# zhihu/ZhiLight

Measured on AMD Instinct MI355X. Metric: decode tokens/s (Llama-3-8B GPTQ-Int4, TP=1 per GPU, batch 1, seq 1024), higher is better.
Workload: dtype f16; 1 GPU; Llama-3-8B GPTQ-Int4 g128 TP=1 batch=1 decode seq=1024 (BASELINE configs[1]); layers=32, parallelism=dp1 (independent TP=1 replicas), global_batch=1, seq_len=1024, valid=True, kv_cache_dtype=fp16, w4_algo=mfma

## Files before the change

### zhilight_amd/build.py

```python
import os
import subprocess
import sys
from concurrent.futures import ThreadPoolExecutor

HERE = os.path.dirname(os.path.abspath(__file__))
CSRC = os.path.join(HERE, "csrc")
OUT = os.path.join(HERE, "libzhilight_amd.so")
HIPCC = os.environ.get("HIPCC", "/opt/rocm/bin/hipcc")
FLAGS = ["--offload-arch=gfx950", "-O3", "-std=c++17", "-fPIC", "-Wall", "-Wno-unused-function",
         "-fno-fast-math", "-ffp-contract=off"]
EXTRA_FLAGS = {"w4_slab.hip": ["-mllvm", "-pragma-unroll-threshold=200000"]}


EXPERIMENTAL = os.environ.get("ZL_BUILD_EXPERIMENTAL", "0") == "1"
EXPERIMENTAL_DIR = os.path.join(HERE, "..", "tools", "experimental")


def sources():
    srcs = sorted(os.path.join(CSRC, f) for f in os.listdir(CSRC) if f.endswith(".hip"))
    if EXPERIMENTAL:
        srcs.append(os.path.join(EXPERIMENTAL_DIR, "w4_engine.hip"))
    return srcs


def _stale(target, deps):
    if not os.path.exists(target):
        return True
    t = os.path.getmtime(target)
    return any(os.path.getmtime(d) > t for d in deps)


def build(force=False, verbose=False):
    srcs = sources()
    hdrs = [os.path.join(CSRC, f) for f in os.listdir(CSRC) if f.endswith(".h")]
    hdrs.append(os.path.join(HERE, "..", "include", "zhilight_amd.h"))
    objdir = os.path.join(HERE, "build")
    os.makedirs(objdir, exist_ok=True)
    flags = FLAGS + (["-DZL_EXPERIMENTAL", "-I" + CSRC] if EXPERIMENTAL else [])
    stamp = os.path.join(objdir, ".flags")
    if not os.path.exists(stamp) or open(stamp).read() != " ".join(flags):
        force = True
    objs = []
    jobs = []
    for s in srcs:
        o = os.path.join(objdir, os.path.basename(s)[:-4] + ".o")
        objs.append(o)
        if force or _stale(o, [s] + hdrs):
            jobs.append([HIPCC] + flags + EXTRA_FLAGS.get(os.path.basename(s), []) + ["-c", s, "-o", o])

    def run(cmd):
        if verbose:
            print(" ".join(cmd), flush=True)
        subprocess.check_call(cmd)

    with ThreadPoolExecutor(max_workers=min(8, max(1, len(jobs)))) as ex:
        list(ex.map(run, jobs))
    if jobs or force or _stale(OUT, objs):
        run([HIPCC, "--offload-arch=gfx950", "-shared", "-fPIC", "-o", OUT] + objs)
    with open(stamp, "w") as fh:
        fh.write(" ".join(flags))
    build_hostcpp(force, verbose)
    build_comm(force, verbose)
    _ref().build(force, verbose)
    return OUT


COMM_OUT = os.path.join(HERE, "libzhilight_amd_comm.so")


def build_comm(force=False, verbose=False):
    src = os.path.join(HERE, "csrc_comm", "comm.hip")
    deps = [src, os.path.join(HERE, "..", "include", "zhilight_amd_comm.h"), os.path.join(HERE, "..", "include", "zhilight_amd.h")]
    if not (force or _stale(COMM_OUT, deps)):
        return COMM_OUT
    rocm = os.environ.get("ROCM_PATH", "/opt/rocm")
    cmd = [HIPCC, "--offload-arch=gfx950", "-O3", "-std=c++17", "-fPIC", "-Wall", "-shared", "-o", COMM_OUT, src,
           "-L" + os.path.join(rocm, "lib"), "-lrccl"]
    if verbose:
        print(" ".join(cmd), flush=True)
    subprocess.check_call(cmd)
    return COMM_OUT


HOSTCPP = os.path.join(HERE, "hostcpp")


HOSTCPP_SOURCES = ("bm_hip.cpp", "bm_layer.cpp", "bm_functions.cpp", "bm_c10d.cpp", "nn_amd.cpp")
HOSTCPP_HEADERS = ("bm_hip.h", "bm_layer.h", "bm_functions.h", "bm_c10d.h", "nn_amd.h")


def hostcpp_target():
    import sysconfig
    return os.path.join(HERE, "zl_internals" + sysconfig.get_config_var("EXT_SUFFIX"))


def build_hostcpp(force=False, verbose=False):
    import pybind11
    import sysconfig
    srcs = [os.path.join(HOSTCPP, f) for f in HOSTCPP_SOURCES + ("py_internals.cpp",)]
    deps = srcs + [os.path.join(HOSTCPP, f) for f in HOSTCPP_HEADERS] + [os.path.join(HERE, "..", "include", "zhilight_amd.h")]
    target = hostcpp_target()
    if not (force or _stale(target, deps)):
        return target
    rocm = os.environ.get("ROCM_PATH", "/opt/rocm")
    cmd = [os.environ.get("CXX", "g++"), "-O2", "-std=c++17", "-fPIC", "-shared", "-D__HIP_PLATFORM_AMD__", "-I" + os.path.join(rocm, "include"),
           "-I" + os.path.join(HERE, "..", "include"), "-I" + pybind11.get_include(), "-I" + sysconfig.get_paths()["include"]] + srcs + [
           "-o", target, "-L" + HERE, "-lzhilight_amd", "-L" + os.path.join(rocm, "lib"), "-lamdhip64",
           "-Wl,-rpath,$ORIGIN", "-Wl,-rpath," + os.path.join(rocm, "lib")]
    if verbose:
        print(" ".join(cmd), flush=True)
    subprocess.check_call(cmd)
    return target


REFERENCE = os.environ.get("ZL_REFERENCE_ROOT", "/root/reference")
ORACLE = os.path.join(os.path.dirname(HERE), "oracle")
_REF_NAMES = ("REFDIR", "REF_TUS", "REF_CHECK_TUS", "REF_CHECK_NAMESPACES", "REF_REPORT_TUS", "REF_CHECK_PENDING",
              "REF_BINDING_TUS", "HOST_SOURCES", "HOST_HEADERS", "HARNESS_SOURCES", "host_target", "refcompile_target",
              "binding_target", "refcheck_report", "build_host", "build_refcompile", "build_binding", "build_refcheck")


def _ref():
    if ORACLE not in sys.path:
        sys.path.insert(0, ORACLE)
    import ref_build
    return ref_build


def __getattr__(name):
    if name in _REF_NAMES:
        return getattr(_ref(), name)
    raise AttributeError("module %r has no attribute %r" % (__name__, name))


if __name__ == "__main__":
    print(build(force="--force" in sys.argv, verbose=True))
```

### zhilight_amd/csrc/attention.hip

```cpp
#include <algorithm>
#include <type_traits>
#include "zl_common.h"

namespace {

constexpr int kSteps = 8;
constexpr int kMaxSplits = 512;

struct AttnParams {
    const uint16_t* q = nullptr;
    const int32_t* buf_lens = nullptr;
    const uint16_t* const* k_bufs = nullptr;
    const uint16_t* const* v_bufs = nullptr;
    const int8_t* mask = nullptr;
    const int32_t* valid_lens = nullptr;
    uint16_t* out = nullptr;
    float* ws = nullptr;
    int b = 0, len_q = 0, h = 0, hkv = 0, n_rep = 0, rows = 0;
    int passes = 0, split_len = 0, max_splits = 0;
    float scale = 0.f;
    int bshd = 0;
    const uint16_t* qkv = nullptr;
    const float* cosv = nullptr;
    const float* sinv = nullptr;
    const int32_t* placement = nullptr;
    uint16_t* const* k_bufs_w = nullptr;
    uint16_t* const* v_bufs_w = nullptr;
    int neox = 1;
    const float* const* k_scales = nullptr;
    const float* const* v_scales = nullptr;
    int half_partials = 0;
    int la = 0;
    int* la_cnt = nullptr;
    int causal = 0;
};

typedef _Float16 hv2 __attribute__((ext_vector_type(2)));

static inline int attn_split_len(int64_t b, int64_t hkv, int64_t max_len) {
    int64_t want = (max_len * b * hkv) / 1024;
    int64_t ls = (want / 128) * 128;
    if (ls < 128) ls = 128;
    if (ls <= 256 && ((max_len + ls - 1) / ls) * b * hkv > 1024) ls += 128;
    if (ls > 2048) ls = 2048;
    while ((max_len + ls - 1) / ls > kMaxSplits && ls < (int64_t)1 << 30) ls += 128;
    return (int)ls;
}

template <int DT>
__device__ __forceinline__ float dot8(const uint4& a, const uint4& b) {
    const uint32_t au[4] = {a.x, a.y, a.z, a.w}, bu[4] = {b.x, b.y, b.z, b.w};
    float acc = 0.f;
#pragma unroll
    for (int e = 0; e < 4; ++e) {
        if constexpr (DT == ZL_F16) {
            acc = __builtin_amdgcn_fdot2(__builtin_bit_cast(hv2, au[e]), __builtin_bit_cast(hv2, bu[e]), acc, false);
        } else {
            acc = __builtin_fmaf(__builtin_bit_cast(float, au[e] << 16), __builtin_bit_cast(float, bu[e] << 16), acc);
            acc = __builtin_fmaf(__builtin_bit_cast(float, au[e] & 0xffff0000u),
                                 __builtin_bit_cast(float, bu[e] & 0xffff0000u), acc);
        }
    }
    return acc;
}

template <int DT>
__device__ __forceinline__ void unpack8(const uint4& v, float (&f)[8]) {
    const uint32_t u[4] = {v.x, v.y, v.z, v.w};
#pragma unroll
    for (int e = 0; e < 4; ++e) {
        f[2 * e] = ZT<DT>::to_f32((uint16_t)(u[e] & 0xffff));
        f[2 * e + 1] = ZT<DT>::to_f32((uint16_t)(u[e] >> 16));
    }
}

template <int DT>
__device__ __forceinline__ uint4 rope8(const uint4& a, const uint4& b, const float* c, const float* s, int d0, int half,
                                       int neox) {
    float af[8], bf[8];
    unpack8<DT>(a, af);
    unpack8<DT>(b, bf);
    uint32_t o[4];
#pragma unroll
    for (int e = 0; e < 8; e += 2) {
        float r[2];
#pragma unroll
        for (int t = 0; t < 2; ++t) {
            const int i = e + t;
            bool minus;
            float partner;
            if (neox) {
                minus = (d0 + i) < half;
                partner = bf[i];
            } else {
                minus = (i & 1) == 0;
                partner = af[i ^ 1];
            }
            r[t] = minus ? __builtin_fmaf(-partner, s[i], af[i] * c[i]) : __builtin_fmaf(partner, s[i], af[i] * c[i]);
        }
        o[e / 2] = (uint32_t)ZT<DT>::from_f32(r[0]) | ((uint32_t)ZT<DT>::from_f32(r[1]) << 16);
    }
    return make_uint4(o[0], o[1], o[2], o[3]);
}

template <int LPK>
__device__ __forceinline__ float key_row_sum(float v) {
#ifdef ZL_ATTN_NO_DPP
#pragma unroll
    for (int off = LPK / 2; off > 0; off >>= 1) v += __shfl_xor(v, off, 64);
    return v;
#endif
    v += __builtin_bit_cast(float, __builtin_amdgcn_update_dpp(0, __builtin_bit_cast(int, v), 0xB1, 0xF, 0xF, false));
    v += __builtin_bit_cast(float, __builtin_amdgcn_update_dpp(0, __builtin_bit_cast(int, v), 0x4E, 0xF, 0xF, false));
    if (LPK >= 8)
        v += __builtin_bit_cast(float, __builtin_amdgcn_update_dpp(0, __builtin_bit_cast(int, v), 0x141, 0xF, 0xF, false));
    if (LPK >= 16)
        v += __builtin_bit_cast(float, __builtin_amdgcn_update_dpp(0, __builtin_bit_cast(int, v), 0x140, 0xF, 0xF, false));
    if (LPK >= 32) v += __shfl_xor(v, 16, 64);
    return v;
}

template <int DT, int D, int RT, bool FUSE, bool MASKED>
__global__ __launch_bounds__(256) void k_decode_attn_partial(const AttnParams p) {
    constexpr int LPK = D / 8;
    constexpr int KPS = 64 / LPK;
    constexpr int CHUNK = KPS * kSteps;
    __shared__ float xw[4][RT][D + 2];

    const int b = blockIdx.z / p.passes, pass = blockIdx.z % p.passes;
    const int hk = blockIdx.y, split = blockIdx.x;
    const int len = p.buf_lens[b];
    const int vlen_in = MASKED ? 0x7fffffff : p.valid_lens[b];
    const uint16_t* kbase = p.k_bufs[b];
    const uint16_t* vbase = p.v_bufs[b];
    const int place = FUSE ? p.placement[b] : -1;
    const int elen = MASKED ? len : min(len, vlen_in);
    const int t0 = split * p.split_len;
    const bool owns_new = FUSE && place >= t0 && place < t0 + p.split_len && place < len;
    if (t0 >= elen && !owns_new) return;
    const int t1 = min(elen, t0 + p.split_len);

    const int lane = threadIdx.x & 63, wave = threadIdx.x >> 6;
    const int grp = lane / LPK, dp = lane % LPK;
    const size_t kv_stride = p.bshd ? (size_t)p.hkv * D : (size_t)D;
    const size_t kv_off = (p.bshd ? (size_t)hk * D : (size_t)hk * len * D) + dp * 8;

    uint4 kk[kSteps], vv[kSteps];
    int c0 = t0 + wave * CHUNK;
    const int last_key = t1 > 0 ? t1 - 1 : 0;
#define ZL_LOAD_CHUNK(base)                                                                      \
    _Pragma("unroll") for (int st = 0; st < kSteps; ++st) {                                      \
        const int key_ = (base) + st * KPS + grp;                                                \
        const int kc_ = key_ < last_key ? key_ : last_key;                                       \
        kk[st] = *reinterpret_cast<const uint4*>(kbase + kv_off + (size_t)kc_ * kv_stride);     \
        vv[st] = *reinterpret_cast<const uint4*>(vbase + kv_off + (size_t)kc_ * kv_stride);     \
    }
    if (len <= 0) return;
    ZL_LOAD_CHUNK(c0)

    size_t mask_off = 0;
    if (MASKED) {
        for (int i = 0; i < b; ++i) mask_off += (size_t)p.buf_lens[i];
        mask_off *= p.len_q;
    }

    uint4 qv[RT];
    int q_of_row[RT];
    uint4 k_new = make_uint4(0, 0, 0, 0), v_new = make_uint4(0, 0, 0, 0);
    if constexpr (FUSE) {
        constexpr int half = D / 2;
        const int d0 = dp * 8;
        const int pd0 = p.neox ? (d0 < half ? d0 + half : d0 - half) : d0;
        float c[8], sn[8];
        const float4* cp = reinterpret_cast<const float4*>(p.cosv + (size_t)b * D + d0);
        const float4* sp = reinterpret_cast<const float4*>(p.sinv + (size_t)b * D + d0);
        const float4 c0v = cp[0], c1v = cp[1], s0v = sp[0], s1v = sp[1];
        c[0] = c0v.x; c[1] = c0v.y; c[2] = c0v.z; c[3] = c0v.w; c[4] = c1v.x; c[5] = c1v.y; c[6] = c1v.z; c[7] = c1v.w;
        sn[0] = s0v.x; sn[1] = s0v.y; sn[2] = s0v.z; sn[3] = s0v.w; sn[4] = s1v.x; sn[5] = s1v.y; sn[6] = s1v.z; sn[7] = s1v.w;
        const uint16_t* row = p.qkv + (size_t)b * (p.h + 2 * p.hkv) * D;
#pragma unroll
        for (int i = 0; i < RT; ++i) {
            qv[i] = make_uint4(0, 0, 0, 0);
            q_of_row[i] = 0;
            const int rr = pass * RT + i;
            if (rr < p.rows) {
                const uint16_t* src = row + (size_t)(hk * p.n_rep + rr) * D;
                qv[i] = rope8<DT>(*reinterpret_cast<const uint4*>(src + d0), *reinterpret_cast<const uint4*>(src + pd0), c, sn,
                                  d0, half, p.neox);
            }
        }
        const uint16_t* ksrc = row + (size_t)(p.h + hk) * D;
        k_new = rope8<DT>(*reinterpret_cast<const uint4*>(ksrc + d0), *reinterpret_cast<const uint4*>(ksrc + pd0), c, sn, d0,
                          half, p.neox);
        v_new = *reinterpret_cast<const uint4*>(row + (size_t)(p.h + p.hkv + hk) * D + d0);
        if (owns_new && pass == 0 && wave == 0 && grp == 0) {
            *reinterpret_cast<uint4*>(p.k_bufs_w[b] + kv_off + (size_t)place * kv_stride) = k_new;
            *reinterpret_cast<uint4*>(p.v_bufs_w[b] + kv_off + (size_t)place * kv_stride) = v_new;
        }
        if (t0 >= elen) return;
    } else {
#pragma unroll
        for (int i = 0; i < RT; ++i) {
            const int rr = pass * RT + i;
            qv[i] = make_uint4(0, 0, 0, 0);
            q_of_row[i] = 0;
            if (rr < p.rows) {
                const int qi = rr / p.n_rep, head = hk * p.n_rep + rr % p.n_rep;
                q_of_row[i] = qi;
                qv[i] = *reinterpret_cast<const uint4*>(p.q + (((size_t)b * p.len_q + qi) * p.h + head) * D + dp * 8);
            }
        }
    }

    float m[RT], l[RT], acc[RT][8];
#pragma unroll
    for (int i = 0; i < RT; ++i) {
        m[i] = -1e20f;
        l[i] = 0.f;
#pragma unroll
        for (int e = 0; e < 8; ++e) acc[i][e] = 0.f;
    }

    while (c0 < t1) {
        float sc[RT][kSteps];
#pragma unroll
        for (int st = 0; st < kSteps; ++st) {
            const int key = c0 + st * KPS + grp;
            if (FUSE && key == place) {
                kk[st] = k_new;
                vv[st] = v_new;
            }
            const bool inb = key < t1;
#pragma unroll
            for (int i = 0; i < RT; ++i) {
                const float d = key_row_sum<LPK>(dot8<DT>(qv[i], kk[st]));
                bool vis = inb;
                if (MASKED) {
                    if (vis) vis = p.mask[mask_off + (size_t)q_of_row[i] * len + key] != 0;
                }
                sc[i][st] = vis ? d * p.scale : -INFINITY;
            }
            if (!inb) vv[st] = make_uint4(0, 0, 0, 0);
        }
#pragma unroll
        for (int i = 0; i < RT; ++i) {
            float mc = sc[i][0];
#pragma unroll
            for (int st = 1; st < kSteps; ++st) mc = fmaxf(mc, sc[i][st]);
            const float mn = fmaxf(m[i], mc);
            const float alpha = __expf(m[i] - mn);
            m[i] = mn;
            l[i] *= alpha;
#pragma unroll
            for (int e = 0; e < 8; ++e) acc[i][e] *= alpha;
        }
#pragma unroll
        for (int st = 0; st < kSteps; ++st) {
            float vf[8];
            unpack8<DT>(vv[st], vf);
            if (MASKED) {
                bool any = false;
#pragma unroll
                for (int i = 0; i < RT; ++i) any = any || (sc[i][st] != -INFINITY);
                if (!any) {
#pragma unroll
                    for (int e = 0; e < 8; ++e) vf[e] = 0.f;
                }
            }
#pragma unroll
            for (int i = 0; i < RT; ++i) {
                const float pr = __expf(sc[i][st] - m[i]);
                l[i] += pr;
#pragma unroll
                for (int e = 0; e < 8; ++e) acc[i][e] = __builtin_fmaf(pr, vf[e], acc[i][e]);
            }
        }
        c0 += 4 * CHUNK;
        if (c0 >= t1) break;
        ZL_LOAD_CHUNK(c0)
    }
#undef ZL_LOAD_CHUNK

#pragma unroll
    for (int off = LPK; off < 64; off <<= 1) {
#pragma unroll
        for (int i = 0; i < RT; ++i) {
            const float m2 = __shfl_xor(m[i], off, 64), l2 = __shfl_xor(l[i], off, 64);
            const float mn = fmaxf(m[i], m2);
            const float f1 = __expf(m[i] - mn), f2 = __expf(m2 - mn);
            l[i] = l[i] * f1 + l2 * f2;
#pragma unroll
            for (int e = 0; e < 8; ++e) {
                const float a2 = __shfl_xor(acc[i][e], off, 64);
                acc[i][e] = acc[i][e] * f1 + a2 * f2;
            }
            m[i] = mn;
        }
    }
    if (grp == 0) {
#pragma unroll
        for (int i = 0; i < RT; ++i) {
#pragma unroll
            for (int e = 0; e < 8; ++e) xw[wave][i][dp * 8 + e] = acc[i][e];
            if (dp == 0) {
                xw[wave][i][D] = m[i];
                xw[wave][i][D + 1] = l[i];
            }
        }
    }
    __syncthreads();
    for (int idx = threadIdx.x; idx < RT * D; idx += 256) {
        const int i = idx / D, d = idx % D;
        const int rr = pass * RT + i;
        if (rr >= p.rows) continue;
        float mn = xw[0][i][D];
#pragma unroll
        for (int w = 1; w < 4; ++w) mn = fmaxf(mn, xw[w][i][D]);
        float a = 0.f, lt = 0.f;
#pragma unroll
        for (int w = 0; w < 4; ++w) {
            const float f = __expf(xw[w][i][D] - mn);
            a = __builtin_fmaf(xw[w][i][d], f, a);
            lt = __builtin_fmaf(xw[w][i][D + 1], f, lt);
        }
        const int qi = rr / p.n_rep, head = hk * p.n_rep + rr % p.n_rep;
        float* dst = p.ws + ((((size_t)b * p.len_q + qi) * p.h + head) * p.max_splits + split) * (D + 2);
        dst[d] = a;
        if (d == 0) {
            dst[D] = mn;
            dst[D + 1] = lt;
        }
    }
}

__device__ __forceinline__ void codes_to_h2(const uint4& w, hv2 (&h)[8]) {
    const uint32_t u[4] = {w.x, w.y, w.z, w.w};
    const hv2 bias = {(_Float16)1152.f, (_Float16)1152.f};
#pragma unroll
    for (int e = 0; e < 4; ++e) {
        h[2 * e] = __builtin_bit_cast(hv2, __builtin_amdgcn_perm(0x64646464u, u[e], 0x04010400u)) - bias;
        h[2 * e + 1] = __builtin_bit_cast(hv2, __builtin_amdgcn_perm(0x64646464u, u[e], 0x04030402u)) - bias;
    }
}
__device__ __forceinline__ void codes_to_f32(const uint4& w, float (&f)[16]) {
    const uint32_t u[4] = {w.x, w.y, w.z, w.w};
#pragma unroll
    for (int e = 0; e < 4; ++e) {
#pragma unroll
        for (int j = 0; j < 4; ++j) f[4 * e + j] = (float)((u[e] >> (8 * j)) & 0xffu) - 128.f;
    }
}

template <int DT, int D, int RT, bool MASKED>
__global__ __launch_bounds__(256) void k_decode_attn_partial_q8(const AttnParams p) {
    constexpr int LPK = D / 16;
    constexpr int KPS = 64 / LPK;
    constexpr int CHUNK = KPS * kSteps;
    constexpr int QW = DT == ZL_F16 ? 8 : 16;
    __shared__ float xw[4][RT][D + 2];

    const int b = blockIdx.z / p.passes, pass = blockIdx.z % p.passes;
    const int hk = blockIdx.y, split = blockIdx.x;
    const int len = p.buf_lens[b];
    const int vlen_in = MASKED ? 0x7fffffff : p.valid_lens[b];
    const uint8_t* kbase = reinterpret_cast<const uint8_t*>(p.k_bufs[b]);
    const uint8_t* vbase = reinterpret_cast<const uint8_t*>(p.v_bufs[b]);
    const float* ksc = p.k_scales[b];
    const float* vsc = p.v_scales[b];
    const int elen = MASKED ? len : min(len, vlen_in);
    const int t0 = split * p.split_len;
    if (t0 >= elen || len <= 0) return;
    const int t1 = min(elen, t0 + p.split_len);

    const int lane = threadIdx.x & 63, wave = threadIdx.x >> 6;
    const int grp = lane / LPK, dp = lane % LPK;
    const size_t kv_stride = p.bshd ? (size_t)p.hkv * D : (size_t)D;
    const size_t kv_off = (p.bshd ? (size_t)hk * D : (size_t)hk * len * D) + dp * 16;
    const size_t sc_stride = p.bshd ? (size_t)p.hkv : 1;
    const size_t sc_off = p.bshd ? (size_t)hk : (size_t)hk * len;

    uint4 kk[kSteps], vv[kSteps];
    float ks[kSteps], vs[kSteps];
    int c0 = t0 + wave * CHUNK;
    const int last_key = t1 - 1;
#define ZL_LOAD_CHUNK_Q8(base)                                                                   \
    _Pragma("unroll") for (int st = 0; st < kSteps; ++st) {                                      \
        const int key_ = (base) + st * KPS + grp;                                                \
        const int kc_ = key_ < last_key ? key_ : last_key;                                       \
        kk[st] = *reinterpret_cast<const uint4*>(kbase + kv_off + (size_t)kc_ * kv_stride);     \
        vv[st] = *reinterpret_cast<const uint4*>(vbase + kv_off + (size_t)kc_ * kv_stride);     \
        ks[st] = ksc[sc_off + (size_t)kc_ * sc_stride];                                          \
        vs[st] = vsc[sc_off + (size_t)kc_ * sc_stride];                                          \
    }
    ZL_LOAD_CHUNK_Q8(c0)

    size_t mask_off = 0;
    if (MASKED) {
        for (int i = 0; i < b; ++i) mask_off += (size_t)p.buf_lens[i];
        mask_off *= p.len_q;
    }

    hv2 qh[RT][8];
    float qf[RT][QW];
    int q_of_row[RT];
#pragma unroll
    for (int i = 0; i < RT; ++i) {
        const int rr = pass * RT + i;
        uint4 lo = make_uint4(0, 0, 0, 0), hi = lo;
        q_of_row[i] = 0;
        if (rr < p.rows) {
            const int qi = rr / p.n_rep, head = hk * p.n_rep + rr % p.n_rep;
            q_of_row[i] = qi;
            const uint16_t* qp = p.q + (((size_t)b * p.len_q + qi) * p.h + head) * D + dp * 16;
            lo = *reinterpret_cast<const uint4*>(qp);
            hi = *reinterpret_cast<const uint4*>(qp + 8);
        }
        if constexpr (DT == ZL_F16) {
            const uint32_t u[8] = {lo.x, lo.y, lo.z, lo.w, hi.x, hi.y, hi.z, hi.w};
#pragma unroll
            for (int e = 0; e < 8; ++e) qh[i][e] = __builtin_bit_cast(hv2, u[e]);
        } else {
            float a[8], c[8];
            unpack8<DT>(lo, a);
            unpack8<DT>(hi, c);
#pragma unroll
            for (int e = 0; e < 8; ++e) {
                qf[i][e] = a[e];
                qf[i][8 + e] = c[e];
            }
        }
    }

    float m[RT], l[RT], acc[RT][16];
#pragma unroll
    for (int i = 0; i < RT; ++i) {
        m[i] = -1e20f;
        l[i] = 0.f;
#pragma unroll
        for (int e = 0; e < 16; ++e) acc[i][e] = 0.f;
    }

    while (c0 < t1) {
        float sc[RT][kSteps];
#pragma unroll
        for (int st = 0; st < kSteps; ++st) {
            const int key = c0 + st * KPS + grp;
            const bool inb = key < t1;
            const float lscale = ks[st] * p.scale;
            hv2 kh[8];
            float kf[16];
            if constexpr (DT == ZL_F16) codes_to_h2(kk[st], kh);
            else codes_to_f32(kk[st], kf);
#pragma unroll
            for (int i = 0; i < RT; ++i) {
                float d = 0.f;
                if constexpr (DT == ZL_F16) {
#pragma unroll
                    for (int e = 0; e < 8; ++e) d = __builtin_amdgcn_fdot2(qh[i][e], kh[e], d, false);
                } else {
#pragma unroll
                    for (int e = 0; e < 16; ++e) d = __builtin_fmaf(qf[i][e], kf[e], d);
                }
                d = key_row_sum<LPK>(d);
                bool vis = inb;
                if (MASKED) {
                    if (vis) vis = p.mask[mask_off + (size_t)q_of_row[i] * len + key] != 0;
                }
                sc[i][st] = vis ? d * lscale : -INFINITY;
            }
            if (!inb) vs[st] = 0.f;
        }
#pragma unroll
        for (int i = 0; i < RT; ++i) {
            float mc = sc[i][0];
#pragma unroll
            for (int st = 1; st < kSteps; ++st) mc = fmaxf(mc, sc[i][st]);
            const float mn = fmaxf(m[i], mc);
            const float alpha = __expf(m[i] - mn);
            m[i] = mn;
            l[i] *= alpha;
#pragma unroll
            for (int e = 0; e < 16; ++e) acc[i][e] *= alpha;
        }
#pragma unroll
        for (int st = 0; st < kSteps; ++st) {
            float vf[16];
            codes_to_f32(vv[st], vf);
            float sv = vs[st];
            if (MASKED) {
                bool any = false;
#pragma unroll
                for (int i = 0; i < RT; ++i) any = any || (sc[i][st] != -INFINITY);
                if (!any) sv = 0.f;
            }
#pragma unroll
            for (int i = 0; i < RT; ++i) {
                const float pr = __expf(sc[i][st] - m[i]);
                l[i] += pr;
                const float w = pr * sv;
#pragma unroll
                for (int e = 0; e < 16; ++e) acc[i][e] = __builtin_fmaf(w, vf[e], acc[i][e]);
            }
        }
        c0 += 4 * CHUNK;
        if (c0 >= t1) break;
        ZL_LOAD_CHUNK_Q8(c0)
    }
#undef ZL_LOAD_CHUNK_Q8

#pragma unroll
    for (int off = LPK; off < 64; off <<= 1) {
#pragma unroll
        for (int i = 0; i < RT; ++i) {
            const float m2 = __shfl_xor(m[i], off, 64), l2 = __shfl_xor(l[i], off, 64);
            const float mn = fmaxf(m[i], m2);
            const float f1 = __expf(m[i] - mn), f2 = __expf(m2 - mn);
            l[i] = l[i] * f1 + l2 * f2;
#pragma unroll
            for (int e = 0; e < 16; ++e) {
                const float a2 = __shfl_xor(acc[i][e], off, 64);
                acc[i][e] = acc[i][e] * f1 + a2 * f2;
            }
            m[i] = mn;
        }
    }
    if (grp == 0) {
#pragma unroll
        for (int i = 0; i < RT; ++i) {
#pragma unroll
            for (int e = 0; e < 16; ++e) xw[wave][i][dp * 16 + e] = acc[i][e];
            if (dp == 0) {
                xw[wave][i][D] = m[i];
                xw[wave][i][D + 1] = l[i];
            }
        }
    }
    __syncthreads();
    for (int idx = threadIdx.x; idx < RT * D; idx += 256) {
        const int i = idx / D, d = idx % D;
        const int rr = pass * RT + i;
        if (rr >= p.rows) continue;
        float mn = xw[0][i][D];
#pragma unroll
        for (int w = 1; w < 4; ++w) mn = fmaxf(mn, xw[w][i][D]);
        float a = 0.f, lt = 0.f;
#pragma unroll
        for (int w = 0; w < 4; ++w) {
            const float f = __expf(xw[w][i][D] - mn);
            a = __builtin_fmaf(xw[w][i][d], f, a);
            lt = __builtin_fmaf(xw[w][i][D + 1], f, lt);
        }
        const int qi = rr / p.n_rep, head = hk * p.n_rep + rr % p.n_rep;
        float* dst = p.ws + ((((size_t)b * p.len_q + qi) * p.h + head) * p.max_splits + split) * (D + 2);
        dst[d] = a;
        if (d == 0) {
            dst[D] = mn;
            dst[D + 1] = lt;
        }
    }
}

typedef _Float16 h8v __attribute__((ext_vector_type(8)));
typedef float f4v __attribute__((ext_vector_type(4)));
typedef short s4v __attribute__((ext_vector_type(4)));
constexpr int kMD = 128;
constexpr int kMVS = kMD + 16;

template <int DT>
__device__ __forceinline__ f4v mfma_t(uint4 a, uint4 b, f4v c) {
    typedef __bf16 b8v __attribute__((ext_vector_type(8)));
    if constexpr (DT == ZL_F16)
        return __builtin_amdgcn_mfma_f32_16x16x32_f16(__builtin_bit_cast(h8v, a), __builtin_bit_cast(h8v, b), c, 0, 0, 0);
    else
        return __builtin_amdgcn_mfma_f32_16x16x32_bf16(__builtin_bit_cast(b8v, a), __builtin_bit_cast(b8v, b), c, 0, 0, 0);
}

#ifndef ZL_LA_BATCH
#define ZL_LA_BATCH 16
#endif
constexpr int kLaBatch = ZL_LA_BATCH;
#ifdef ZL_ATTN_PROBE
__device__ unsigned long long* zl_aprobe_p = nullptr;
#define ZL_APROBE_INIT()                                                                                           \
    unsigned long long* ap_ = nullptr;                                                                             \
    {                                                                                                              \
        const unsigned wg_ = (blockIdx.z * gridDim.y + blockIdx.y) * gridDim.x + blockIdx.x;                        \
        if (zl_aprobe_p && (threadIdx.x & 63) == 0 && wg_ < 8192) ap_ = zl_aprobe_p + ((size_t)wg_ * 8 + (threadIdx.x >> 6)) * 8; \
    }
#define ZL_APROBE(slot) do { if (ap_) ap_[slot] = wall_clock64(); } while (0)
#else
#define ZL_APROBE_INIT() do {} while (0)
#define ZL_APROBE(slot) do {} while (0)
#endif
constexpr int kLaMaxSplits = 64;

template <int DT>
__device__ __forceinline__ void attn_tail_la(const AttnParams& p, float* xw, int b, int hk, int split, int nw, int ns, unsigned long long* ap_) {
    (void)ap_;
    constexpr int WS = 16 * (kMD + 2);
    const int nthr = nw * 64;
    const bool direct = ns == 1;
    const size_t stat0 = (size_t)p.b * p.len_q * p.h * p.max_splits * (kMD / 2);
    for (int it = threadIdx.x; it < p.rows * (kMD / 4); it += nthr) {
        const int i = it / (kMD / 4), d0 = (it % (kMD / 4)) * 4;
        const float* src = xw + (size_t)i * (kMD + 2);
        float mn = src[kMD];
        for (int w = 1; w < nw; ++w) mn = fmaxf(mn, src[w * WS + kMD]);
        float a[4] = {0.f, 0.f, 0.f, 0.f}, lt = 0.f;
        for (int w = 0; w < nw; ++w) {
            const float f = __expf(src[w * WS + kMD] - mn);
            typedef float f2v __attribute__((ext_vector_type(2)));
            const f2v v01 = *reinterpret_cast<const f2v*>(src + w * WS + d0), v23 = *reinterpret_cast<const f2v*>(src + w * WS + d0 + 2);
            const f4v v = (f4v){v01[0], v01[1], v23[0], v23[1]};
#pragma unroll
            for (int e = 0; e < 4; ++e) a[e] = __builtin_fmaf(v[e], f, a[e]);
            lt = __builtin_fmaf(src[w * WS + kMD + 1], f, lt);
        }
        const int qi = i / p.n_rep, head = hk * p.n_rep + i % p.n_rep;
        const size_t vh = ((size_t)b * p.len_q + qi) * p.h + head;
        const size_t rec = vh * p.max_splits + split;
        if (direct) {
            uint16_t o4[4];
#pragma unroll
            for (int e = 0; e < 4; ++e) {
                float ov;
                if (p.half_partials) ov = ((float)(_Float16)(a[e] / lt) * lt) * (1.0f / (lt + 1e-20f));
                else ov = a[e] / (lt + 1e-20f);
                o4[e] = ZT<DT>::from_f32(ov);
            }
            *reinterpret_cast<uint2*>(p.out + vh * kMD + d0) = make_uint2((uint32_t)o4[0] | ((uint32_t)o4[1] << 16), (uint32_t)o4[2] | ((uint32_t)o4[3] << 16));
            continue;
        }
        auto st8 = [](void* dst, uint32_t lo, uint32_t hi) {
            __hip_atomic_store(reinterpret_cast<uint64_t*>(dst), (uint64_t)lo | ((uint64_t)hi << 32), __ATOMIC_RELAXED, __HIP_MEMORY_SCOPE_AGENT);
        };
        if (p.half_partials) {
            uint32_t w2[2];
#pragma unroll
            for (int e = 0; e < 2; ++e)
                w2[e] = (uint32_t)__builtin_bit_cast(uint16_t, (_Float16)(a[2 * e] / lt)) | ((uint32_t)__builtin_bit_cast(uint16_t, (_Float16)(a[2 * e + 1] / lt)) << 16);
            st8(reinterpret_cast<uint16_t*>(p.ws) + rec * kMD + d0, w2[0], w2[1]);
            if (d0 == 0) st8(p.ws + stat0 + rec * 2, __builtin_bit_cast(uint32_t, mn), __builtin_bit_cast(uint32_t, lt));
        } else {
            float* dst = p.ws + rec * (kMD + 2) + d0;
            st8(dst, __builtin_bit_cast(uint32_t, a[0]), __builtin_bit_cast(uint32_t, a[1]));
            st8(dst + 2, __builtin_bit_cast(uint32_t, a[2]), __builtin_bit_cast(uint32_t, a[3]));
            if (d0 == 0) st8(dst + kMD, __builtin_bit_cast(uint32_t, mn), __builtin_bit_cast(uint32_t, lt));
        }
    }
    if (direct) return;
#if defined(__HIP_DEVICE_COMPILE__) && !defined(__gfx950__)
#error "attn_tail_la's hand-off is written for gfx950 (vmcnt-tracked write-through stores); revisit it for any other target"
#endif
    asm volatile("s_waitcnt vmcnt(0)" ::: "memory");
    __syncthreads();
    ZL_APROBE(5);
    int* flag = reinterpret_cast<int*>(xw);
    if (threadIdx.x == 0) {
        int* cnt = p.la_cnt + (size_t)b * p.hkv + hk;
        const int old = __hip_atomic_fetch_add(cnt, 1, __ATOMIC_RELAXED, __HIP_MEMORY_SCOPE_AGENT);
        if (old == ns - 1) __hip_atomic_store(cnt, 0, __ATOMIC_RELAXED, __HIP_MEMORY_SCOPE_AGENT);
        *flag = old == ns - 1;
    }
    __syncthreads();
    ZL_APROBE(6);
    if (!*flag) return;
    for (int it = threadIdx.x; it < p.rows * (kMD / 4); it += nthr) {
        const int i = it / (kMD / 4), d0 = (it % (kMD / 4)) * 4;
        const int qi = i / p.n_rep, head = hk * p.n_rep + i % p.n_rep;
        const size_t vh = ((size_t)b * p.len_q + qi) * p.h + head;
        float mn = -1e20f, a[4] = {0.f, 0.f, 0.f, 0.f}, z = 0.f;
        for (int u0 = 0; u0 < ns; u0 += kLaBatch) {
            uint64_t lo[kLaBatch], hi[kLaBatch], ml[kLaBatch];
#pragma unroll
            for (int j = 0; j < kLaBatch; ++j) {
                const size_t rec = vh * p.max_splits + min(u0 + j, ns - 1);
                if (p.half_partials) {
                    lo[j] = __hip_atomic_load(reinterpret_cast<const uint64_t*>(reinterpret_cast<const uint16_t*>(p.ws) + (rec * kMD + d0)),
                                              __ATOMIC_RELAXED, __HIP_MEMORY_SCOPE_AGENT);
                    hi[j] = 0;
                    ml[j] = __hip_atomic_load(reinterpret_cast<const uint64_t*>(p.ws + stat0 + rec * 2), __ATOMIC_RELAXED, __HIP_MEMORY_SCOPE_AGENT);
                } else {
                    const uint64_t* src = reinterpret_cast<const uint64_t*>(p.ws + rec * (kMD + 2) + d0);
                    lo[j] = __hip_atomic_load(src, __ATOMIC_RELAXED, __HIP_MEMORY_SCOPE_AGENT);
                    hi[j] = __hip_atomic_load(src + 1, __ATOMIC_RELAXED, __HIP_MEMORY_SCOPE_AGENT);
                    ml[j] = __hip_atomic_load(reinterpret_cast<const uint64_t*>(p.ws + rec * (kMD + 2) + kMD), __ATOMIC_RELAXED, __HIP_MEMORY_SCOPE_AGENT);
                }
            }
            float mb = mn;
#pragma unroll
            for (int j = 0; j < kLaBatch; ++j)
                if (u0 + j < ns) mb = fmaxf(mb, __builtin_bit_cast(float, (uint32_t)ml[j]));
            if (u0 > 0) {
                const float r = __expf(mn - mb);
#pragma unroll
                for (int e = 0; e < 4; ++e) a[e] *= r;
                z *= r;
            }
            mn = mb;
#pragma unroll
            for (int j = 0; j < kLaBatch; ++j) {
                if (u0 + j < ns) {
                    const float ms = __builtin_bit_cast(float, (uint32_t)ml[j]), ls = __builtin_bit_cast(float, (uint32_t)(ml[j] >> 32));
                    if (p.half_partials) {
                        const float f = ls * __expf(ms - mn);
#pragma unroll
                        for (int e = 0; e < 4; ++e)
                            a[e] = __builtin_fmaf((float)__builtin_bit_cast(_Float16, (uint16_t)(lo[j] >> (16 * e))), f, a[e]);
                        z += f;
                    } else {
                        const float f = __expf(ms - mn);
                        a[0] = __builtin_fmaf(__builtin_bit_cast(float, (uint32_t)lo[j]), f, a[0]);
                        a[1] = __builtin_fmaf(__builtin_bit_cast(float, (uint32_t)(lo[j] >> 32)), f, a[1]);
                        a[2] = __builtin_fmaf(__builtin_bit_cast(float, (uint32_t)hi[j]), f, a[2]);
                        a[3] = __builtin_fmaf(__builtin_bit_cast(float, (uint32_t)(hi[j] >> 32)), f, a[3]);
                        z = __builtin_fmaf(ls, f, z);
                    }
                }
            }
        }
        uint16_t o4[4];
        const float zi = 1.0f / (z + 1e-20f);
#pragma unroll
        for (int e = 0; e < 4; ++e) o4[e] = ZT<DT>::from_f32(p.half_partials ? a[e] * zi : a[e] / (z + 1e-20f));
        *reinterpret_cast<uint2*>(p.out + vh * kMD + d0) = make_uint2((uint32_t)o4[0] | ((uint32_t)o4[1] << 16), (uint32_t)o4[2] | ((uint32_t)o4[3] << 16));
    }
    ZL_APROBE(7);
}

#ifndef ZL_ATTN8_WAVES_PER_SIMD
#define ZL_ATTN8_WAVES_PER_SIMD 2
#endif
#define ZL_ATTN8_OCC(NW_) ((NW_) == 4 ? 4 : ZL_ATTN8_WAVES_PER_SIMD)
template <int DT, int NW = 4, bool LA = false, int PF = 1, bool MASKED = false, bool CAUSAL = false>
__global__ __launch_bounds__(64 * NW, PF >= 3 ? 1 : (PF == 2 || MASKED) ? 2 : ZL_ATTN8_OCC(NW)) void k_decode_attn_mfma(const AttnParams p) {
    static_assert(!MASKED || (!LA && PF == 1), "the mask form exists for the two-launch route only");
    static_assert(!CAUSAL || (!LA && PF == 1 && !MASKED && NW == 4), "the causal form exists for the two-launch route only");
    __shared__ __attribute__((aligned(16))) uint16_t vs[NW][32 * kMVS];
    const int b = blockIdx.z, hk = CAUSAL ? (int)(blockIdx.y % (unsigned)p.hkv) : (int)blockIdx.y, split = blockIdx.x;
    const int row0 = CAUSAL ? 16 * (int)(blockIdx.y / (unsigned)p.hkv) : 0;
    const int nrows = CAUSAL ? min(16, p.rows - row0) : p.rows;
    const int len = p.buf_lens[b];
    const int vlen_in = MASKED ? 0x7fffffff : CAUSAL ? p.valid_lens[b] + (row0 + nrows - 1) / p.n_rep : p.valid_lens[b];
    const int8_t* mrow = nullptr;
    if constexpr (MASKED) {
        size_t mask_off = 0;
        for (int i = 0; i < b; ++i) mask_off += (size_t)p.buf_lens[i];
        mrow = p.mask + mask_off;
    }
    const uint16_t* kbase = p.k_bufs[b];
    const uint16_t* vbase = p.v_bufs[b];
    const int elen = min(len, vlen_in);
    const int t0 = split * p.split_len;
    const int nw = LA ? __builtin_amdgcn_readfirstlane((int)(blockDim.x >> 6)) : NW;
    ZL_APROBE_INIT();
    ZL_APROBE(0);
    if (t0 >= elen || len <= 0) {
        if constexpr (LA) {
            if (split == 0)
                for (int idx = threadIdx.x; idx < p.rows * kMD; idx += nw * 64) {
                    const int i = idx / kMD, qi = i / p.n_rep, head = hk * p.n_rep + i % p.n_rep;
                    p.out[(((size_t)b * p.len_q + qi) * p.h + head) * kMD + idx % kMD] = 0;
                }
        }
        return;
    }
    const int t1 = min(elen, t0 + p.split_len);
    const int last_key = t1 - 1;

    const int lane = threadIdx.x & 63, wave = threadIdx.x >> 6;
    const int r = lane & 15, kq = lane >> 4;
    const size_t kv_stride = p.bshd ? (size_t)p.hkv * kMD : (size_t)kMD;
    const size_t kv_off = p.bshd ? (size_t)hk * kMD : (size_t)hk * len * kMD;

    uint4 kkA[2][4], kkB[PF >= 2 ? 2 : 1][4], kkC[PF >= 3 ? 2 : 1][4];
    uint4 vA0, vA1, vA2, vA3, vA4, vA5, vA6, vA7, vB0, vB1, vB2, vB3, vB4, vB5, vB6, vB7, vC0, vC1, vC2, vC3, vC4, vC5, vC6, vC7;
    int c0 = t0 + wave * 32;
    const int cstep = nw * 32;
#define ZL_MFMA_LOAD_K(KK, base)                                                                                  \
    _Pragma("unroll") for (int blk_ = 0; blk_ < 2; ++blk_) {                                                   \
        const int key_ = (base) + 16 * blk_ + r;                                                               \
        const uint16_t* src_ = kbase + kv_off + (size_t)(key_ < last_key ? key_ : last_key) * kv_stride + 8 * kq; \
        _Pragma("unroll") for (int t_ = 0; t_ < 4; ++t_) KK[blk_][t_] = *reinterpret_cast<const uint4*>(src_ + 32 * t_); \
    }
#define ZL_MFMA_V1(VS, j_, base)                                                                                 \
    {                                                                                                          \
        const int key_ = (base) + 4 * j_ + (lane >> 4);                                                        \
        VS##j_ = *reinterpret_cast<const uint4*>(vbase + kv_off + (size_t)(key_ < last_key ? key_ : last_key) * kv_stride + (lane & 15) * 8); \
    }
#define ZL_MFMA_LOAD_V(VS, base)                                                                               \
    ZL_MFMA_V1(VS, 0, base) ZL_MFMA_V1(VS, 1, base) ZL_MFMA_V1(VS, 2, base) ZL_MFMA_V1(VS, 3, base) ZL_MFMA_V1(VS, 4, base) \
    ZL_MFMA_V1(VS, 5, base) ZL_MFMA_V1(VS, 6, base) ZL_MFMA_V1(VS, 7, base)
    int mbA = 1, mbX = 1;
#define ZL_MFMA_LOAD_M(MB, base)                                                                               \
    if constexpr (MASKED) {                                                                                    \
        const int key_ = (base) + (lane & 31);                                                                 \
        MB = mrow[key_ < last_key ? key_ : last_key];                                                          \
    }
    ZL_MFMA_LOAD_M(mbA, c0)
    ZL_MFMA_LOAD_K(kkA, c0)
    ZL_MFMA_LOAD_V(vA, c0)
    if constexpr (PF >= 2) {
        ZL_MFMA_LOAD_K(kkB, c0 + cstep)
        ZL_MFMA_LOAD_V(vB, c0 + cstep)
    }
    if constexpr (PF >= 3) {
        ZL_MFMA_LOAD_K(kkC, c0 + 2 * cstep)
        ZL_MFMA_LOAD_V(vC, c0 + 2 * cstep)
    }
    ZL_APROBE(1);

    uint4 qf[4];
    int rlim = t1;
    {
        uint4 z = make_uint4(0, 0, 0, 0);
        const bool live = r < nrows;
        const int rr = row0 + (live ? r : 0);
        const int qi = rr / p.n_rep, head = hk * p.n_rep + rr % p.n_rep;
        if constexpr (CAUSAL) rlim = min(t1, p.valid_lens[b] + qi);
        const uint16_t* qp = p.q + (((size_t)b * p.len_q + qi) * p.h + head) * kMD + 8 * kq;
#pragma unroll
        for (int t = 0; t < 4; ++t) {
            uint4 v = *reinterpret_cast<const uint4*>(qp + 32 * t);
            qf[t] = live ? v : z;
        }
    }

    f4v o[8];
#pragma unroll
    for (int db = 0; db < 8; ++db) o[db] = (f4v){0.f, 0.f, 0.f, 0.f};
    float m_run = -1e20f, l_run = 0.f;
    uint16_t* vsw = vs[wave];
    const uint16_t* vtr = vsw + (4 * kq + (r >> 2)) * kMVS + 4 * (r & 3);

    if (c0 >= t1) c0 = -1;
    auto chunk = [&](uint4 (&KK)[2][4], uint4& v0, uint4& v1, uint4& v2, uint4& v3, uint4& v4, uint4& v5, uint4& v6, uint4& v7,
                     int& MB, const int cur) __attribute__((always_inline)) {
        uint32_t vbits = 0xffffffffu;
        if constexpr (MASKED) {
            vbits = (uint32_t)__ballot(lane < 32 && MB != 0 && cur + lane < t1);
            const int vsh = lane >> 4;
#define ZL_MFMA_VZ(j_) if (!((vbits >> (4 * j_ + vsh)) & 1u)) v##j_ = make_uint4(0, 0, 0, 0);
            ZL_MFMA_VZ(0) ZL_MFMA_VZ(1) ZL_MFMA_VZ(2) ZL_MFMA_VZ(3) ZL_MFMA_VZ(4) ZL_MFMA_VZ(5) ZL_MFMA_VZ(6) ZL_MFMA_VZ(7)
#undef ZL_MFMA_VZ
        }
        f4v st[2];
#pragma unroll
        for (int blk = 0; blk < 2; ++blk) {
            st[blk] = (f4v){0.f, 0.f, 0.f, 0.f};
#pragma unroll
            for (int t = 0; t < 4; ++t)
                st[blk] = mfma_t<DT>(KK[blk][t], qf[t], st[blk]);
        }
        {
            uint16_t* vdst = vsw + (lane >> 4) * kMVS + (lane & 15) * 8;
#define ZL_MFMA_VST(j_) *reinterpret_cast<uint4*>(vdst + 4 * j_ * kMVS) = v##j_;
            ZL_MFMA_VST(0) ZL_MFMA_VST(1) ZL_MFMA_VST(2) ZL_MFMA_VST(3) ZL_MFMA_VST(4) ZL_MFMA_VST(5) ZL_MFMA_VST(6) ZL_MFMA_VST(7)
#undef ZL_MFMA_VST
        }
        ZL_MFMA_LOAD_M(MB, cur + PF * cstep)
        ZL_MFMA_LOAD_K(KK, cur + PF * cstep)
        ZL_MFMA_LOAD_V(v, cur + PF * cstep)
        float sv[2][4];
        float mloc = -INFINITY;
#pragma unroll
        for (int blk = 0; blk < 2; ++blk) {
#pragma unroll
            for (int i = 0; i < 4; ++i) {
                const int key = cur + 16 * blk + 4 * kq + i;
                bool vis = key < (CAUSAL ? rlim : t1);
                if constexpr (MASKED) vis = (vbits >> (16 * blk + 4 * kq + i)) & 1u;
                sv[blk][i] = vis ? st[blk][i] * p.scale : -INFINITY;
                mloc = fmaxf(mloc, sv[blk][i]);
            }
        }
        mloc = fmaxf(mloc, __shfl_xor(mloc, 16, 64));
        mloc = fmaxf(mloc, __shfl_xor(mloc, 32, 64));
        const float m_new = fmaxf(m_run, mloc);
        const float alpha = __expf(m_run - m_new);
#ifdef ZL_ATTN_PROBE
        if (m_run == -1e20f && m_new > -1e19f) ZL_APROBE(2);
#endif
        m_run = m_new;
        float pr[2][4];
        float lsum = 0.f;
#pragma unroll
        for (int blk = 0; blk < 2; ++blk) {
#pragma unroll
            for (int i = 0; i < 4; ++i) {
                pr[blk][i] = __expf(sv[blk][i] - m_new);
                lsum += pr[blk][i];
            }
        }
        auto cvt = [](float x) -> uint16_t {
            if constexpr (DT == ZL_F16) return __builtin_bit_cast(uint16_t, (_Float16)x);
            else {
                uint32_t u = __builtin_bit_cast(uint32_t, x);
                return (uint16_t)((u + 0x7fffu + ((u >> 16) & 1u)) >> 16);
            }
        };
        auto hi_lo = [&](float a, float b2, uint32_t& hw, uint32_t& lw) {
            const uint16_t ah = cvt(a), bh = cvt(b2);
            hw = (uint32_t)ah | ((uint32_t)bh << 16);
            lw = (uint32_t)cvt(a - ZT<DT>::to_f32(ah)) | ((uint32_t)cvt(b2 - ZT<DT>::to_f32(bh)) << 16);
        };
        uint4 pf, pl;
        hi_lo(pr[0][0], pr[0][1], pf.x, pl.x);
        hi_lo(pr[0][2], pr[0][3], pf.y, pl.y);
        hi_lo(pr[1][0], pr[1][1], pf.z, pl.z);
        hi_lo(pr[1][2], pr[1][3], pf.w, pl.w);
        l_run = l_run * alpha + lsum;
#pragma unroll
        for (int db = 0; db < 8; ++db) {
            o[db][0] *= alpha; o[db][1] *= alpha; o[db][2] *= alpha; o[db][3] *= alpha;
        }
#pragma unroll
        for (int db = 0; db < 8; ++db) {
            const s4v lo = __builtin_amdgcn_ds_read_tr16_b64_v4i16((__attribute__((address_space(3))) s4v*)(vtr + 16 * db));
            const s4v hi = __builtin_amdgcn_ds_read_tr16_b64_v4i16((__attribute__((address_space(3))) s4v*)(vtr + 16 * kMVS + 16 * db));
            typedef short s8v __attribute__((ext_vector_type(8)));
            const s8v a = __builtin_shufflevector(lo, hi, 0, 1, 2, 3, 4, 5, 6, 7);
            o[db] = mfma_t<DT>(__builtin_bit_cast(uint4, a), pf, o[db]);
            o[db] = mfma_t<DT>(__builtin_bit_cast(uint4, a), pl, o[db]);
        }
    };
    while (c0 >= 0) {
        chunk(kkA, vA0, vA1, vA2, vA3, vA4, vA5, vA6, vA7, mbA, c0);
        c0 += cstep;
        if (c0 >= t1) break;
        if constexpr (PF >= 2) {
            chunk(kkB, vB0, vB1, vB2, vB3, vB4, vB5, vB6, vB7, mbX, c0);
            c0 += cstep;
            if (c0 >= t1) break;
        }
        if constexpr (PF >= 3) {
            chunk(kkC, vC0, vC1, vC2, vC3, vC4, vC5, vC6, vC7, mbX, c0);
            c0 += cstep;
            if (c0 >= t1) break;
        }
    }
#undef ZL_MFMA_LOAD_K
#undef ZL_MFMA_LOAD_V
#undef ZL_MFMA_LOAD_M
#undef ZL_MFMA_V1

    ZL_APROBE(3);
    l_run += __shfl_xor(l_run, 16, 64);
    l_run += __shfl_xor(l_run, 32, 64);
    __syncthreads();
    float* xw = reinterpret_cast<float*>(&vs[0][0]);
    if (r < nrows) {
        float* dst = xw + ((size_t)wave * 16 + r) * (kMD + 2);
#pragma unroll
        for (int db = 0; db < 8; ++db) *reinterpret_cast<f4v*>(dst + 16 * db + 4 * kq) = o[db];
        if (kq == 0) {
            dst[kMD] = m_run;
            dst[kMD + 1] = l_run;
        }
    }
    __syncthreads();
    if constexpr (LA) {
        ZL_APROBE(4);
#ifdef ZL_ATTN_PROBE
        attn_tail_la<DT>(p, xw, b, hk, split, nw, (elen + p.split_len - 1) / p.split_len, ap_);
#else
        attn_tail_la<DT>(p, xw, b, hk, split, nw, (elen + p.split_len - 1) / p.split_len, nullptr);
#endif
        return;
    }
    for (int idx = threadIdx.x; idx < nrows * kMD; idx += NW * 64) {
        const int i = idx / kMD, d = idx % kMD;
        const float* src = xw + (size_t)i * (kMD + 2);
        constexpr int WS = 16 * (kMD + 2);
        float mn = src[kMD];
#pragma unroll
        for (int w = 1; w < NW; ++w) mn = fmaxf(mn, src[w * WS + kMD]);
        float a = 0.f, lt = 0.f;
#pragma unroll
        for (int w = 0; w < NW; ++w) {
            const float f = __expf(src[w * WS + kMD] - mn);
            a = __builtin_fmaf(src[w * WS + d], f, a);
            lt = __builtin_fmaf(src[w * WS + kMD + 1], f, lt);
        }
        const int qi = (row0 + i) / p.n_rep, head = hk * p.n_rep + (row0 + i) % p.n_rep;
        const size_t rec = (((size_t)b * p.len_q + qi) * p.h + head) * p.max_splits + split;
        if (p.half_partials) {
            uint16_t* hp = reinterpret_cast<uint16_t*>(p.ws);
            hp[rec * kMD + d] = __builtin_bit_cast(uint16_t, (_Float16)((MASKED && lt == 0.f) ? 0.f : a / lt));
            if (d == 0) {
                float* st = p.ws + (size_t)p.b * p.len_q * p.h * p.max_splits * (kMD / 2) + rec * 2;
                st[0] = mn;
                st[1] = lt;
            }
            continue;
        }
        float* dst = p.ws + rec * (kMD + 2);
        dst[d] = a;
        if (d == 0) {
            dst[kMD] = mn;
            dst[kMD + 1] = lt;
        }
    }
}

__global__ __launch_bounds__(256, 3) void k_decode_attn_mfma_q8(const AttnParams p) {
    __shared__ __attribute__((aligned(16))) uint16_t vs[4][32 * kMVS];
    const int b = blockIdx.z, hk = blockIdx.y, split = blockIdx.x;
    const int len = p.buf_lens[b];
    const int vlen_in = p.valid_lens[b];
    const uint8_t* kbase = reinterpret_cast<const uint8_t*>(p.k_bufs[b]);
    const uint8_t* vbase = reinterpret_cast<const uint8_t*>(p.v_bufs[b]);
    const float* ksc = p.k_scales[b];
    const float* vsc = p.v_scales[b];
    const int elen = min(len, vlen_in);
    const int t0 = split * p.split_len;
    if (t0 >= elen || len <= 0) return;
    const int t1 = min(elen, t0 + p.split_len);
    const int last_key = t1 - 1;

    const int lane = threadIdx.x & 63, wave = threadIdx.x >> 6;
    const int r = lane & 15, kq = lane >> 4;
    const size_t kv_stride = p.bshd ? (size_t)p.hkv * kMD : (size_t)kMD;
    const size_t kv_off = p.bshd ? (size_t)hk * kMD : (size_t)hk * len * kMD;
    const size_t sc_stride = p.bshd ? (size_t)p.hkv : 1;
    const size_t sc_off = p.bshd ? (size_t)hk : (size_t)hk * len;

    uint4 kk[2][2], vv0, vv1, vv2, vv3;
    float ksv[2][4], vsv[2][4];
    int c0 = t0 + wave * 32;
#define ZL_Q8_LOAD_K(base)                                                                                     \
    _Pragma("unroll") for (int blk_ = 0; blk_ < 2; ++blk_) {                                                   \
        const int key_ = (base) + 16 * blk_ + r;                                                               \
        const uint8_t* src_ = kbase + kv_off + (size_t)(key_ < last_key ? key_ : last_key) * kv_stride + 16 * kq; \
        kk[blk_][0] = *reinterpret_cast<const uint4*>(src_);                                                   \
        kk[blk_][1] = *reinterpret_cast<const uint4*>(src_ + 64);                                              \
        _Pragma("unroll") for (int i_ = 0; i_ < 4; ++i_) {                                                     \
            const int ks_ = (base) + 16 * blk_ + 4 * kq + i_;                                                  \
            const size_t so_ = sc_off + (size_t)(ks_ < last_key ? ks_ : last_key) * sc_stride;                 \
            ksv[blk_][i_] = ksc[so_];                                                                          \
            vsv[blk_][i_] = vsc[so_];                                                                          \
        }                                                                                                      \
    }
#define ZL_Q8_V1(j_, base)                                                                                     \
    {                                                                                                          \
        const int key_ = (base) + 8 * j_ + (lane >> 3);                                                        \
        vv##j_ = *reinterpret_cast<const uint4*>(vbase + kv_off + (size_t)(key_ < last_key ? key_ : last_key) * kv_stride + (lane & 7) * 16); \
    }
#define ZL_Q8_LOAD_V(base) ZL_Q8_V1(0, base) ZL_Q8_V1(1, base) ZL_Q8_V1(2, base) ZL_Q8_V1(3, base)
    ZL_Q8_LOAD_K(c0)
    ZL_Q8_LOAD_V(c0)

    h8v qf[4];
    {
        uint4 z = make_uint4(0, 0, 0, 0);
        const bool live = r < p.rows;
        const int rr = live ? r : 0;
        const int qi = rr / p.n_rep, head = hk * p.n_rep + rr % p.n_rep;
        const uint16_t* qp = p.q + (((size_t)b * p.len_q + qi) * p.h + head) * kMD + 16 * kq;
#pragma unroll
        for (int t = 0; t < 4; ++t) {
            uint4 v = *reinterpret_cast<const uint4*>(qp + 64 * (t >> 1) + 8 * (t & 1));
            qf[t] = __builtin_bit_cast(h8v, live ? v : z);
        }
    }

    f4v o[8];
#pragma unroll
    for (int db = 0; db < 8; ++db) o[db] = (f4v){0.f, 0.f, 0.f, 0.f};
    float m_run = -1e20f, l_run = 0.f;
    uint16_t* vsw = vs[wave];
    const uint16_t* vtr = vsw + (4 * kq + (r >> 2)) * kMVS + 4 * (r & 3);
    const hv2 bias = {(_Float16)1152.f, (_Float16)1152.f};
    auto cvt8 = [&](uint32_t w0, uint32_t w1) {
        uint4 o4;
        o4.x = __builtin_bit_cast(uint32_t, __builtin_bit_cast(hv2, __builtin_amdgcn_perm(0x64646464u, w0, 0x04010400u)) - bias);
        o4.y = __builtin_bit_cast(uint32_t, __builtin_bit_cast(hv2, __builtin_amdgcn_perm(0x64646464u, w0, 0x04030402u)) - bias);
        o4.z = __builtin_bit_cast(uint32_t, __builtin_bit_cast(hv2, __builtin_amdgcn_perm(0x64646464u, w1, 0x04010400u)) - bias);
        o4.w = __builtin_bit_cast(uint32_t, __builtin_bit_cast(hv2, __builtin_amdgcn_perm(0x64646464u, w1, 0x04030402u)) - bias);
        return o4;
    };

    if (c0 >= t1) c0 = -1;
    while (c0 >= 0) {
        f4v st[2];
        float ks_cur[2][4], vs_cur[2][4];
#pragma unroll
        for (int blk = 0; blk < 2; ++blk) {
            st[blk] = (f4v){0.f, 0.f, 0.f, 0.f};
#pragma unroll
            for (int u = 0; u < 2; ++u) {
                const uint4 c = kk[blk][u];
                st[blk] = __builtin_amdgcn_mfma_f32_16x16x32_f16(__builtin_bit_cast(h8v, cvt8(c.x, c.y)), qf[2 * u], st[blk], 0, 0, 0);
                st[blk] = __builtin_amdgcn_mfma_f32_16x16x32_f16(__builtin_bit_cast(h8v, cvt8(c.z, c.w)), qf[2 * u + 1], st[blk], 0, 0, 0);
            }
#pragma unroll
            for (int i = 0; i < 4; ++i) {
                ks_cur[blk][i] = ksv[blk][i];
                vs_cur[blk][i] = vsv[blk][i];
            }
        }
        {
            uint16_t* vdst = vsw + (lane >> 3) * kMVS + (lane & 7) * 16;
#define ZL_Q8_VST(j_)                                                                                          \
            *reinterpret_cast<uint4*>(vdst + 8 * j_ * kMVS) = cvt8(vv##j_.x, vv##j_.y);                        \
            *reinterpret_cast<uint4*>(vdst + 8 * j_ * kMVS + 8) = cvt8(vv##j_.z, vv##j_.w);
            ZL_Q8_VST(0) ZL_Q8_VST(1) ZL_Q8_VST(2) ZL_Q8_VST(3)
#undef ZL_Q8_VST
        }
        const int cur = c0;
        c0 += 4 * 32;
        ZL_Q8_LOAD_K(c0)
        ZL_Q8_LOAD_V(c0)
        float sv[2][4];
        float mloc = -INFINITY;
#pragma unroll
        for (int blk = 0; blk < 2; ++blk) {
#pragma unroll
            for (int i = 0; i < 4; ++i) {
                const int key = cur + 16 * blk + 4 * kq + i;
                sv[blk][i] = key < t1 ? st[blk][i] * (ks_cur[blk][i] * p.scale) : -INFINITY;
                mloc = fmaxf(mloc, sv[blk][i]);
            }
        }
        mloc = fmaxf(mloc, __shfl_xor(mloc, 16, 64));
        mloc = fmaxf(mloc, __shfl_xor(mloc, 32, 64));
        const float m_new = fmaxf(m_run, mloc);
        const float alpha = __expf(m_run - m_new);
        m_run = m_new;
        h8v pf, pl;
        float lsum = 0.f;
#pragma unroll
        for (int blk = 0; blk < 2; ++blk) {
#pragma unroll
            for (int i = 0; i < 4; ++i) {
                const int key = cur + 16 * blk + 4 * kq + i;
                const float pr = __expf(sv[blk][i] - m_new);
                lsum += pr;
                const float pw = key < t1 ? pr * vs_cur[blk][i] : 0.f;
                const _Float16 ph = (_Float16)pw;
                pf[blk * 4 + i] = ph;
                pl[blk * 4 + i] = (_Float16)(pw - (float)ph);
            }
        }
        l_run = l_run * alpha + lsum;
#pragma unroll
        for (int db = 0; db < 8; ++db) {
            o[db][0] *= alpha; o[db][1] *= alpha; o[db][2] *= alpha; o[db][3] *= alpha;
        }
#pragma unroll
        for (int db = 0; db < 8; ++db) {
            const s4v lo = __builtin_amdgcn_ds_read_tr16_b64_v4i16((__attribute__((address_space(3))) s4v*)(vtr + 16 * db));
            const s4v hi = __builtin_amdgcn_ds_read_tr16_b64_v4i16((__attribute__((address_space(3))) s4v*)(vtr + 16 * kMVS + 16 * db));
            typedef short s8v __attribute__((ext_vector_type(8)));
            const s8v a = __builtin_shufflevector(lo, hi, 0, 1, 2, 3, 4, 5, 6, 7);
            o[db] = __builtin_amdgcn_mfma_f32_16x16x32_f16(__builtin_bit_cast(h8v, a), pf, o[db], 0, 0, 0);
            o[db] = __builtin_amdgcn_mfma_f32_16x16x32_f16(__builtin_bit_cast(h8v, a), pl, o[db], 0, 0, 0);
        }
        if (c0 >= t1) break;
    }
#undef ZL_Q8_LOAD_K
#undef ZL_Q8_LOAD_V
#undef ZL_Q8_V1

    l_run += __shfl_xor(l_run, 16, 64);
    l_run += __shfl_xor(l_run, 32, 64);
    __syncthreads();
    float* xw = reinterpret_cast<float*>(&vs[0][0]);
    if (r < p.rows) {
        float* dst = xw + ((size_t)wave * 16 + r) * (kMD + 2);
#pragma unroll
        for (int db = 0; db < 8; ++db) *reinterpret_cast<f4v*>(dst + 16 * db + 4 * kq) = o[db];
        if (kq == 0) {
            dst[kMD] = m_run;
            dst[kMD + 1] = l_run;
        }
    }
    __syncthreads();
    for (int idx = threadIdx.x; idx < p.rows * kMD; idx += 256) {
        const int i = idx / kMD, d = idx % kMD;
        const float* src = xw + (size_t)i * (kMD + 2);
        constexpr int WS = 16 * (kMD + 2);
        float mn = src[kMD];
#pragma unroll
        for (int w = 1; w < 4; ++w) mn = fmaxf(mn, src[w * WS + kMD]);
        float a = 0.f, lt = 0.f;
#pragma unroll
        for (int w = 0; w < 4; ++w) {
            const float f = __expf(src[w * WS + kMD] - mn);
            a = __builtin_fmaf(src[w * WS + d], f, a);
            lt = __builtin_fmaf(src[w * WS + kMD + 1], f, lt);
        }
        const int qi = i / p.n_rep, head = hk * p.n_rep + i % p.n_rep;
        float* dst = p.ws + ((((size_t)b * p.len_q + qi) * p.h + head) * p.max_splits + split) * (kMD + 2);
        dst[d] = a;
        if (d == 0) {
            dst[kMD] = mn;
            dst[kMD + 1] = lt;
        }
    }
}

template <int DT, int D>
__global__ void k_decode_attn_combine(const AttnParams p) {
    constexpr int kMaxS = 512;
    __shared__ float sf[kMaxS];
    __shared__ float red[16];
    const int vh = blockIdx.x;
    const int b = vh / (p.len_q * p.h);
    const int len = p.buf_lens[b];
    const int vlen_in = p.valid_lens ? p.valid_lens[b] + (p.causal ? (vh / p.h) % p.len_q : 0) : 0x7fffffff;
    const int elen = p.mask ? len : min(len, vlen_in);
    const int ns = min((elen + p.split_len - 1) / p.split_len, kMaxS);
    const int d = threadIdx.x;
    const float* src = p.ws + (size_t)vh * p.max_splits * (D + 2);
    if (ns <= 16) {
        float v[16];
#pragma unroll
        for (int u = 0; u < 16; ++u) v[u] = src[(size_t)min(u, max(ns - 1, 0)) * (D + 2) + d];
        if (d < ns) {
            sf[d] = src[(size_t)d * (D + 2) + D];
            sf[64 + d] = src[(size_t)d * (D + 2) + D + 1];
        }
        __syncthreads();
        float mn = -1e20f;
        for (int s = 0; s < ns; ++s) mn = fmaxf(mn, sf[s]);
        float a = 0.f, z = 0.f;
#pragma unroll
        for (int u = 0; u < 16; ++u) {
            if (u < ns) {
                const float f = __expf(sf[u] - mn);
                a = __builtin_fmaf(v[u], f, a);
                z = __builtin_fmaf(sf[64 + u], f, z);
            }
        }
        p.out[(size_t)vh * D + d] = ZT<DT>::from_f32(a / (z + 1e-20f));
        return;
    }
    float mloc = -1e20f;
    for (int s = d; s < ns; s += D) {
        const float ms = src[(size_t)s * (D + 2) + D];
        sf[s] = ms;
        mloc = fmaxf(mloc, ms);
    }
    const float mn = zl_block_max(mloc, red);
    float zloc = 0.f;
    for (int s = d; s < ns; s += D) {
        const float f = __expf(sf[s] - mn);
        sf[s] = f;
        zloc = __builtin_fmaf(src[(size_t)s * (D + 2) + D + 1], f, zloc);
    }
    const float z = zl_block_sum(zloc, red);
    float a = 0.f;
    int s = 0;
    for (; s + 4 <= ns; s += 4) {
        const float v0 = src[(size_t)(s + 0) * (D + 2) + d], v1 = src[(size_t)(s + 1) * (D + 2) + d];
        const float v2 = src[(size_t)(s + 2) * (D + 2) + d], v3 = src[(size_t)(s + 3) * (D + 2) + d];
        a = __builtin_fmaf(v0, sf[s], a);
        a = __builtin_fmaf(v1, sf[s + 1], a);
        a = __builtin_fmaf(v2, sf[s + 2], a);
        a = __builtin_fmaf(v3, sf[s + 3], a);
    }
    for (; s < ns; ++s) a = __builtin_fmaf(src[(size_t)s * (D + 2) + d], sf[s], a);
    p.out[(size_t)vh * D + d] = ZT<DT>::from_f32(a / (z + 1e-20f));
}

__global__ __launch_bounds__(kMD) void k_decode_attn_combine_h(const AttnParams p) {
    const int vh = blockIdx.x, b = vh / p.h, d = threadIdx.x;
    const int len = p.buf_lens[b];
    const int elen = p.valid_lens ? min(len, p.valid_lens[b]) : len;
    const int ns = min((elen + p.split_len - 1) / p.split_len, p.max_splits);
    const uint16_t* part = reinterpret_cast<const uint16_t*>(p.ws) + (size_t)vh * p.max_splits * kMD;
    const float2* stat = reinterpret_cast<const float2*>(p.ws + (size_t)p.b * p.h * p.max_splits * (kMD / 2)) + (size_t)vh * p.max_splits;
    float mn = -1e20f;
    for (int u = 0; u < ns; ++u) mn = fmaxf(mn, stat[u].x);
    float a = 0.f, z = 0.f;
    for (int u = 0; u < ns; ++u) {
        const float2 st = stat[u];
        const float f = st.y * __expf(st.x - mn);
        a = __builtin_fmaf((float)__builtin_bit_cast(_Float16, part[(size_t)u * kMD + d]), f, a);
        z += f;
    }
    const float zi = 1.0f / (z + 1e-20f);
    p.out[(size_t)vh * kMD + d] = __builtin_bit_cast(uint16_t, zl_f32_to_f16(a * zi));
}

#define ZL_ATTN_TRY(...)                 \
    do {                                \
        const int e_ = (__VA_ARGS__);   \
        if (e_) return e_;              \
    } while (0)

template <class F>
static inline int by_dtype(int dtype, F&& f) {
    return dtype == ZL_F16 ? f(std::integral_constant<int, ZL_F16>{}) : f(std::integral_constant<int, ZL_BF16>{});
}

static inline int attn_check_args(bool pointers, int64_t b, int64_t len_q, int64_t h, int64_t hkv, int64_t d, int64_t max_len_buf) {
    ZL_CHECK_ARG(pointers, ZL_EINVAL);
    ZL_CHECK_ARG(b > 0 && len_q > 0 && h > 0 && hkv > 0 && d > 0 && max_len_buf > 0, ZL_EINVAL);
    ZL_CHECK_ARG(h % hkv == 0, ZL_ESHAPE);
    return ZL_OK;
}

static inline bool attn_dtype_ok(int dtype) { return dtype == ZL_F16 || dtype == ZL_BF16; }

static inline bool attn_mfma_shape_ok(int64_t b, int64_t h, int64_t hkv, int64_t d) {
    return d == kMD && h / hkv <= 16 && b <= 65535 && hkv <= 65535;
}

static int attn_geometry(AttnParams& p, int64_t b, int64_t len_q, int64_t h, int64_t hkv, int64_t max_len_buf,
                         int cap = kMaxSplits, int split_len = 0) {
    p.b = (int)b; p.len_q = (int)len_q; p.h = (int)h; p.hkv = (int)hkv; p.n_rep = (int)(h / hkv);
    p.rows = p.len_q * p.n_rep;
    p.split_len = split_len ? split_len : attn_split_len(b, hkv, max_len_buf);
    p.max_splits = (int)((max_len_buf + p.split_len - 1) / p.split_len);
    return p.max_splits <= cap ? ZL_OK : ZL_ELIMIT;
}

static int attn_set_passes(AttnParams& p, int rt) {
    p.passes = (p.rows + rt - 1) / rt;
    return (int64_t)p.b * p.passes <= 65535 && p.hkv <= 65535 ? ZL_OK : ZL_ELIMIT;
}

template <int NW = 4, bool LA = false, int PF = 1, bool MASKED = false, bool CAUSAL = false>
int launch_mfma(const AttnParams& p, int dtype, hipStream_t st, int waves = NW) {
    const int tiles = CAUSAL ? (p.rows + 15) / 16 : 1;
    const dim3 grid((unsigned)p.max_splits, (unsigned)(p.hkv * tiles), (unsigned)p.b);
    return by_dtype(dtype, [&](auto dt) {
        hipLaunchKernelGGL((k_decode_attn_mfma<decltype(dt)::value, NW, LA, PF, MASKED, CAUSAL>), grid, dim3(64 * waves), 0, st, p);
        return zl_launch_status();
    });
}

template <int D>
int launch_combine(const AttnParams& p, int dtype, hipStream_t st) {
    return by_dtype(dtype, [&](auto dt) {
        hipLaunchKernelGGL((k_decode_attn_combine<decltype(dt)::value, D>), dim3((unsigned)((int64_t)p.b * p.len_q * p.h)), dim3(D), 0, st, p);
        return zl_launch_status();
    });
}

static inline int valu_rt(int rows) { return rows >= 8 ? 8 : (rows >= 4 ? 4 : (rows >= 2 ? 2 : 1)); }
static inline int q8_rt(int rows) { return rows >= 4 ? 4 : (rows >= 2 ? 2 : 1); }

template <int DT, int D, bool FUSE>
int launch_d(const AttnParams& p, hipStream_t st) {
    dim3 grid((unsigned)p.max_splits, (unsigned)p.hkv, (unsigned)(p.b * p.passes));
#define ZL_ATTN_RT(RT)                                                                                          \
    if (p.mask) hipLaunchKernelGGL((k_decode_attn_partial<DT, D, RT, FUSE, true>), grid, dim3(256), 0, st, p);      \
    else hipLaunchKernelGGL((k_decode_attn_partial<DT, D, RT, FUSE, false>), grid, dim3(256), 0, st, p);
    switch (valu_rt(p.rows)) {
        case 1: ZL_ATTN_RT(1) break;
        case 2: ZL_ATTN_RT(2) break;
        case 4: ZL_ATTN_RT(4) break;
        default: ZL_ATTN_RT(8) break;
    }
#undef ZL_ATTN_RT
    ZL_ATTN_TRY(zl_launch_status());
    return launch_combine<D>(p, DT, st);
}

template <int DT, int D>
int launch_q8(const AttnParams& p, hipStream_t st) {
    dim3 grid((unsigned)p.max_splits, (unsigned)p.hkv, (unsigned)(p.b * p.passes));
#define ZL_ATTN_RT(RT)                                                                                       \
    if (p.mask) hipLaunchKernelGGL((k_decode_attn_partial_q8<DT, D, RT, true>), grid, dim3(256), 0, st, p);  \
    else hipLaunchKernelGGL((k_decode_attn_partial_q8<DT, D, RT, false>), grid, dim3(256), 0, st, p);
    switch (q8_rt(p.rows)) {
        case 1: ZL_ATTN_RT(1) break;
        case 2: ZL_ATTN_RT(2) break;
        default: ZL_ATTN_RT(4) break;
    }
#undef ZL_ATTN_RT
    ZL_ATTN_TRY(zl_launch_status());
    return launch_combine<D>(p, DT, st);
}

template <bool FUSE>
int launch_valu(const AttnParams& p, int64_t d, int dtype, hipStream_t st) {
    return by_dtype(dtype, [&](auto dt) -> int {
        constexpr int DT = decltype(dt)::value;
        switch (d) {
            case 64: return launch_d<DT, 64, FUSE>(p, st);
            case 128: return launch_d<DT, 128, FUSE>(p, st);
            case 256: return launch_d<DT, 256, FUSE>(p, st);
            default: return ZL_ESHAPE;
        }
    });
}

int launch_valu_q8(const AttnParams& p, int64_t d, int dtype, hipStream_t st) {
    return by_dtype(dtype, [&](auto dt) -> int {
        constexpr int DT = decltype(dt)::value;
        switch (d) {
            case 64: return launch_q8<DT, 64>(p, st);
            case 128: return launch_q8<DT, 128>(p, st);
            case 256: return launch_q8<DT, 256>(p, st);
            default: return ZL_ESHAPE;
        }
    });
}

int attn_splits(const uint16_t* q, const int32_t* buf_lens, const uint16_t* const* k_bufs, const uint16_t* const* v_bufs,
                const int8_t* mask, const int32_t* valid_lens, void* workspace, int64_t b, int64_t h, int64_t hkv, int64_t d,
                float scale, int64_t max_len_buf, int bshd, int dtype, int half_partials, zl_stream_t s) {
    ZL_ATTN_TRY(attn_check_args(q && buf_lens && k_bufs && v_bufs && (mask || valid_lens) && workspace, b, 1, h, hkv, d, max_len_buf));
    ZL_CHECK_ARG(attn_mfma_shape_ok(b, h, hkv, d), ZL_ESHAPE);
    ZL_CHECK_ARG(attn_dtype_ok(dtype), ZL_EDTYPE);
    AttnParams p;
    p.q = q; p.buf_lens = buf_lens; p.k_bufs = k_bufs; p.v_bufs = v_bufs; p.mask = mask; p.valid_lens = valid_lens;
    p.ws = (float*)workspace; p.scale = scale; p.bshd = bshd; p.passes = 1; p.half_partials = half_partials;
    ZL_ATTN_TRY(attn_geometry(p, b, 1, h, hkv, max_len_buf));
    return mask ? launch_mfma<4, false, 1, true>(p, dtype, (hipStream_t)s) : launch_mfma<>(p, dtype, (hipStream_t)s);
}

}

extern "C" {

int64_t zl_decode_attn_workspace_bytes(int64_t b, int64_t len_q, int64_t h, int64_t d, int64_t max_len_buf) {
    if (b <= 0 || len_q <= 0 || h <= 0 || d <= 0 || max_len_buf <= 0) return ZL_EINVAL;
    int64_t splits = (max_len_buf + 127) / 128;
    return b * len_q * h * splits * (d + 2) * 4;
}

int zl_decode_attn(const uint16_t* q, const int32_t* buf_lens, const uint16_t* const* k_bufs,
                   const uint16_t* const* v_bufs, const int8_t* mask, const int32_t* valid_lens, uint16_t* out,
                   void* workspace, int64_t b, int64_t len_q, int64_t h, int64_t hkv, int64_t d, float scale,
                   int64_t max_len_buf, int bshd, int dtype, zl_stream_t s) {
    return zl_decode_attn_ex(q, buf_lens, k_bufs, v_bufs, mask, valid_lens, out, workspace, b, len_q, h, hkv, d, scale, max_len_buf,
                             bshd, dtype, 0, s);
}

int zl_decode_attn_ex(const uint16_t* q, const int32_t* buf_lens, const uint16_t* const* k_bufs,
                      const uint16_t* const* v_bufs, const int8_t* mask, const int32_t* valid_lens, uint16_t* out,
                      void* workspace, int64_t b, int64_t len_q, int64_t h, int64_t hkv, int64_t d, float scale,
                      int64_t max_len_buf, int bshd, int dtype, int algo, zl_stream_t s) {
    ZL_ATTN_TRY(attn_check_args(q && buf_lens && k_bufs && v_bufs && out && workspace && (mask || valid_lens), b, len_q, h, hkv, d,
                                max_len_buf));
    ZL_CHECK_ARG(attn_dtype_ok(dtype), ZL_EDTYPE);
    AttnParams p;
    p.q = q; p.buf_lens = buf_lens; p.k_bufs = k_bufs; p.v_bufs = v_bufs; p.mask = mask; p.valid_lens = valid_lens;
    p.out = out; p.ws = (float*)workspace; p.scale = scale; p.bshd = bshd;
    ZL_ATTN_TRY(attn_geometry(p, b, len_q, h, hkv, max_len_buf));
    ZL_ATTN_TRY(attn_set_passes(p, valu_rt(p.rows)));
    hipStream_t hs = (hipStream_t)s;
    if (algo != 1 && (!mask || (len_q == 1 && !valid_lens)) && d == kMD && p.rows <= 16) {
        p.passes = 1;
        ZL_ATTN_TRY(mask ? launch_mfma<4, false, 1, true>(p, dtype, hs) : launch_mfma<>(p, dtype, hs));
        return launch_combine<kMD>(p, dtype, hs);
    }
    return launch_valu<false>(p, d, dtype, hs);
}

int zl_decode_attn_causal(const uint16_t* q, const int32_t* buf_lens, const uint16_t* const* k_bufs, const uint16_t* const* v_bufs,
                          const int32_t* valid_lens, uint16_t* out, void* workspace, int64_t b, int64_t len_q, int64_t h, int64_t hkv,
                          int64_t d, float scale, int64_t max_len_buf, int bshd, int dtype, zl_stream_t s) {
    ZL_ATTN_TRY(attn_check_args(q && buf_lens && k_bufs && v_bufs && valid_lens && out && workspace, b, len_q, h, hkv, d, max_len_buf));
    ZL_CHECK_ARG(d == kMD, ZL_ESHAPE);
    ZL_CHECK_ARG(attn_dtype_ok(dtype), ZL_EDTYPE);
    ZL_CHECK_ARG(len_q <= 32, ZL_ELIMIT);
    AttnParams p;
    p.q = q; p.buf_lens = buf_lens; p.k_bufs = k_bufs; p.v_bufs = v_bufs; p.valid_lens = valid_lens;
    p.out = out; p.ws = (float*)workspace; p.scale = scale; p.bshd = bshd; p.passes = 1; p.causal = 1;
    ZL_ATTN_TRY(attn_geometry(p, b, len_q, h, hkv, max_len_buf));
    const int64_t tiles = (p.rows + 15) / 16;
    ZL_CHECK_ARG(b <= 65535 && hkv * tiles <= 65535 && b * len_q * h < ((int64_t)1 << 31), ZL_ELIMIT);
    ZL_ATTN_TRY(launch_mfma<4, false, 1, false, true>(p, dtype, (hipStream_t)s));
    return launch_combine<kMD>(p, dtype, (hipStream_t)s);
}

int64_t zl_decode_attn_split_len(int64_t b, int64_t hkv, int64_t max_len_buf) {
    if (b <= 0 || hkv <= 0 || max_len_buf <= 0) return ZL_EINVAL;
    return attn_split_len(b, hkv, max_len_buf);
}

int zl_decode_attn_splits(const uint16_t* q, const int32_t* buf_lens, const uint16_t* const* k_bufs,
                          const uint16_t* const* v_bufs, const int32_t* valid_lens, void* workspace, int64_t b, int64_t h,
                          int64_t hkv, int64_t d, float scale, int64_t max_len_buf, int bshd, int dtype, zl_stream_t s) {
    return attn_splits(q, buf_lens, k_bufs, v_bufs, nullptr, valid_lens, workspace, b, h, hkv, d, scale, max_len_buf, bshd, dtype, 0, s);
}

int zl_decode_attn_splits_h(const uint16_t* q, const int32_t* buf_lens, const uint16_t* const* k_bufs,
                            const uint16_t* const* v_bufs, const int32_t* valid_lens, void* workspace, int64_t b, int64_t h,
                            int64_t hkv, int64_t d, float scale, int64_t max_len_buf, int bshd, zl_stream_t s) {
    return attn_splits(q, buf_lens, k_bufs, v_bufs, nullptr, valid_lens, workspace, b, h, hkv, d, scale, max_len_buf, bshd, ZL_F16, 1, s);
}

int zl_decode_attn_splits_h_mask(const uint16_t* q, const int32_t* buf_lens, const uint16_t* const* k_bufs,
                                 const uint16_t* const* v_bufs, const int8_t* mask, void* workspace, int64_t b, int64_t h,
                                 int64_t hkv, int64_t d, float scale, int64_t max_len_buf, int bshd, zl_stream_t s) {
    return attn_splits(q, buf_lens, k_bufs, v_bufs, mask, nullptr, workspace, b, h, hkv, d, scale, max_len_buf, bshd, ZL_F16, 1, s);
}

int zl_decode_attn_combine_h(const void* workspace, const int32_t* buf_lens, const int32_t* valid_lens, uint16_t* out, int64_t b,
                             int64_t h, int64_t hkv, int64_t max_len_buf, zl_stream_t s) {
    ZL_CHECK_ARG(workspace && buf_lens && out, ZL_EINVAL);
    ZL_CHECK_ARG(b > 0 && h > 0 && hkv > 0 && max_len_buf > 0, ZL_EINVAL);
    AttnParams p;
    p.buf_lens = buf_lens; p.valid_lens = valid_lens; p.out = out; p.ws = (float*)const_cast<void*>(workspace);
    ZL_ATTN_TRY(attn_geometry(p, b, 1, h, hkv, max_len_buf));
    hipLaunchKernelGGL(k_decode_attn_combine_h, dim3((unsigned)(b * h)), dim3(kMD), 0, (hipStream_t)s, p);
    return zl_launch_status();
}

static inline int la_split_len(int64_t b, int64_t hkv, int64_t max_len) {
    int64_t ls = attn_split_len(b, hkv, max_len);
    int cus = zl_device_cu_count();
    if (cus <= 0) cus = 256;
    const int64_t pairs = b * hkv;
    if (pairs * 4 >= cus && max_len <= 16384) {
        const int64_t splits = pairs >= cus ? 1 : (cus + pairs - 1) / pairs;
        ls = ((max_len + splits - 1) / splits + 31) / 32 * 32;
        if (ls < 128) ls = 128;
    }
    while ((max_len + ls - 1) / ls > kLaMaxSplits) ls += 128;
    return (int)ls;
}

int64_t zl_decode_attn_la_split_len(int64_t b, int64_t hkv, int64_t max_len_buf) {
    if (b <= 0 || hkv <= 0 || max_len_buf <= 0) return ZL_EINVAL;
    return la_split_len(b, hkv, max_len_buf);
}

static inline int64_t la_counter_bytes(int64_t b, int64_t hkv) { return (b * hkv * 4 + 255) / 256 * 256; }

int64_t zl_decode_attn_la_workspace_bytes(int64_t b, int64_t h, int64_t hkv, int64_t max_len_buf, int64_t split_len) {
    if (b <= 0 || h <= 0 || hkv <= 0 || max_len_buf <= 0 || split_len < 0 || split_len % 32 != 0) return ZL_EINVAL;
    int64_t splits = split_len ? (max_len_buf + split_len - 1) / split_len : std::min<int64_t>(kLaMaxSplits, (max_len_buf + 31) / 32);
    if (splits > kLaMaxSplits) return ZL_ELIMIT;
    return la_counter_bytes(b, hkv) + b * h * splits * (kMD + 2) * 4;
}

int zl_decode_attn_la(const uint16_t* q, const int32_t* buf_lens, const uint16_t* const* k_bufs, const uint16_t* const* v_bufs,
                      const int32_t* valid_lens, uint16_t* out, void* workspace, int64_t b, int64_t h, int64_t hkv, int64_t d,
                      float scale, int64_t max_len_buf, int bshd, int dtype, int64_t split_len, int half_partials, zl_stream_t s) {
    ZL_ATTN_TRY(attn_check_args(q && buf_lens && k_bufs && v_bufs && valid_lens && out && workspace, b, 1, h, hkv, d, max_len_buf));
    ZL_CHECK_ARG(attn_mfma_shape_ok(b, h, hkv, d), ZL_ESHAPE);
    ZL_CHECK_ARG(attn_dtype_ok(dtype), ZL_EDTYPE);
    ZL_CHECK_ARG(!(half_partials & 1) || dtype == ZL_F16, ZL_EDTYPE);
    ZL_CHECK_ARG(split_len >= 0 && split_len % 32 == 0, ZL_EINVAL);
    AttnParams p;
    p.q = q; p.buf_lens = buf_lens; p.k_bufs = k_bufs; p.v_bufs = v_bufs; p.valid_lens = valid_lens; p.out = out;
    p.la = 1; p.la_cnt = reinterpret_cast<int*>(workspace);
    p.ws = reinterpret_cast<float*>(reinterpret_cast<char*>(workspace) + la_counter_bytes(b, hkv));
    p.scale = scale; p.bshd = bshd; p.passes = 1; p.half_partials = half_partials & 1;
    ZL_ATTN_TRY(attn_geometry(p, b, 1, h, hkv, max_len_buf, kLaMaxSplits, split_len ? (int)split_len : la_split_len(b, hkv, max_len_buf)));
    ZL_CHECK_ARG((int64_t)b * h * p.max_splits * (kMD + 2) * 4 < ((int64_t)1 << 31), ZL_ELIMIT);
    int nw = p.split_len >= 128 ? 4 : p.split_len / 32;
    const int nw_req = (half_partials >> 8) & 0xff;
    if (nw_req == 1 || nw_req == 2 || nw_req == 4 || nw_req == 8) nw = nw_req * 32 <= p.split_len ? nw_req : nw;
    if (nw == 8) return launch_mfma<8, true>(p, dtype, (hipStream_t)s);
#ifndef ZL_ATTN_LA_PF
#define ZL_ATTN_LA_PF 2
#endif
    return launch_mfma<4, true, ZL_ATTN_LA_PF>(p, dtype, (hipStream_t)s, nw);
}

int zl_decode_attn_fused(const float* cosv, const float* sinv, const uint16_t* qkv, const int32_t* placement,
                         const int32_t* buf_lens, const int32_t* valid_lens, uint16_t* const* k_bufs,
                         uint16_t* const* v_bufs, uint16_t* out, void* workspace, int64_t b, int64_t h, int64_t hkv,
                         int64_t d, float scale, int64_t max_len_buf, int neox, int bshd, int dtype, zl_stream_t s) {
    ZL_ATTN_TRY(attn_check_args(cosv && sinv && qkv && placement && buf_lens && valid_lens && k_bufs && v_bufs && out && workspace, b, 1, h,
                                hkv, d, max_len_buf));
    ZL_CHECK_ARG(attn_dtype_ok(dtype), ZL_EDTYPE);
    AttnParams p;
    p.buf_lens = buf_lens; p.valid_lens = valid_lens; p.out = out; p.ws = (float*)workspace; p.scale = scale; p.bshd = bshd;
    p.k_bufs = reinterpret_cast<const uint16_t* const*>(k_bufs);
    p.v_bufs = reinterpret_cast<const uint16_t* const*>(v_bufs);
    p.qkv = qkv; p.cosv = cosv; p.sinv = sinv; p.placement = placement; p.k_bufs_w = k_bufs; p.v_bufs_w = v_bufs; p.neox = neox;
    ZL_ATTN_TRY(attn_geometry(p, b, 1, h, hkv, max_len_buf));
    ZL_ATTN_TRY(attn_set_passes(p, valu_rt(p.rows)));
    return launch_valu<true>(p, d, dtype, (hipStream_t)s);
}

int zl_decode_attn_quant(const uint16_t* q, const int32_t* buf_lens, const uint8_t* const* k_bufs,
                         const uint8_t* const* v_bufs, const float* const* k_scales, const float* const* v_scales,
                         const int8_t* mask, const int32_t* valid_lens, uint16_t* out, void* workspace, int64_t b,
                         int64_t len_q, int64_t h, int64_t hkv, int64_t d, float scale, int64_t max_len_buf, int bshd,
                         int dtype, zl_stream_t s) {
    return zl_decode_attn_quant_ex(q, buf_lens, k_bufs, v_bufs, k_scales, v_scales, mask, valid_lens, out, workspace, b, len_q, h, hkv,
                                   d, scale, max_len_buf, bshd, dtype, 0, s);
}

int zl_decode_attn_quant_ex(const uint16_t* q, const int32_t* buf_lens, const uint8_t* const* k_bufs,
                         const uint8_t* const* v_bufs, const float* const* k_scales, const float* const* v_scales,
                         const int8_t* mask, const int32_t* valid_lens, uint16_t* out, void* workspace, int64_t b,
                         int64_t len_q, int64_t h, int64_t hkv, int64_t d, float scale, int64_t max_len_buf, int bshd,
                         int dtype, int algo, zl_stream_t s) {
    ZL_ATTN_TRY(attn_check_args(q && buf_lens && k_bufs && v_bufs && k_scales && v_scales && out && workspace && (mask || valid_lens), b,
                                len_q, h, hkv, d, max_len_buf));
    ZL_CHECK_ARG(attn_dtype_ok(dtype), ZL_EDTYPE);
    AttnParams p;
    p.q = q; p.buf_lens = buf_lens; p.mask = mask; p.valid_lens = valid_lens; p.out = out; p.ws = (float*)workspace;
    p.k_bufs = reinterpret_cast<const uint16_t* const*>(k_bufs);
    p.v_bufs = reinterpret_cast<const uint16_t* const*>(v_bufs);
    p.k_scales = k_scales; p.v_scales = v_scales; p.scale = scale; p.bshd = bshd;
    ZL_ATTN_TRY(attn_geometry(p, b, len_q, h, hkv, max_len_buf));
    ZL_ATTN_TRY(attn_set_passes(p, q8_rt(p.rows)));
    hipStream_t hs = (hipStream_t)s;
    if (algo != 1 && !mask && dtype == ZL_F16 && d == kMD && p.rows <= 16) {
        p.passes = 1;
        hipLaunchKernelGGL(k_decode_attn_mfma_q8, dim3((unsigned)p.max_splits, (unsigned)hkv, (unsigned)b), dim3(256), 0, hs, p);
        ZL_ATTN_TRY(zl_launch_status());
        return launch_combine<kMD>(p, dtype, hs);
    }
    return launch_valu_q8(p, d, dtype, hs);
}

}

#ifdef ZL_ATTN_PROBE
extern "C" int zl_debug_set_attn_probe(void* p) { return (int)hipMemcpyToSymbol(HIP_SYMBOL(zl_aprobe_p), &p, sizeof(p)); }
#endif
```

### zhilight_amd/csrc/dense_gemv.hip

```cpp
#include "zl_common.h"
#include "zl_stage.h"

namespace {

constexpr int kRing = 8;

struct DenseParams {
    const uint16_t* x;
    int64_t ldx;
    const uint16_t* w;
    const uint16_t* bias;
    uint16_t* y;
    const uint16_t* norm_w;
    float norm_eps, alpha;
    int m, n, k, kp;
    int loads_per_row;
    int rows_per_wave;
    float2* argmax_ws;
    int total_waves;
};

typedef _Float16 hv2 __attribute__((ext_vector_type(2)));

template <int DT>
__device__ __forceinline__ float dot8(uint4 a, uint4 b, float acc) {
    const uint32_t au[4] = {a.x, a.y, a.z, a.w}, bu[4] = {b.x, b.y, b.z, b.w};
#pragma unroll
    for (int e = 0; e < 4; ++e) {
        if constexpr (DT == ZL_F16) {
            acc = __builtin_amdgcn_fdot2(__builtin_bit_cast(hv2, au[e]), __builtin_bit_cast(hv2, bu[e]), acc, false);
        } else {
            acc = __builtin_fmaf(__builtin_bit_cast(float, au[e] << 16), __builtin_bit_cast(float, bu[e] << 16), acc);
            acc = __builtin_fmaf(__builtin_bit_cast(float, au[e] & 0xffff0000u),
                                 __builtin_bit_cast(float, bu[e] & 0xffff0000u), acc);
        }
    }
    return acc;
}

template <int DT, int MT>
__global__ __launch_bounds__(256) void k_dense_gemv(const DenseParams p) {
    extern __shared__ __attribute__((aligned(16))) unsigned char smem[];
    uint16_t* xs = reinterpret_cast<uint16_t*>(smem);
    float* red = reinterpret_cast<float*>(smem + (size_t)MT * p.kp * 2);

    const int lane = threadIdx.x & 63;
    const int wave = __builtin_amdgcn_readfirstlane(threadIdx.x >> 6);
    const int m0 = blockIdx.y * MT;
    const int L = p.loads_per_row;
    const int gw = blockIdx.x * 4 + wave;
    const int row0 = gw * p.rows_per_wave;
    int nrows = p.n - row0;
    nrows = nrows < 0 ? 0 : (nrows > p.rows_per_wave ? p.rows_per_wave : nrows);
    const int total = nrows * L;

    uint4 wq[kRing];
    int iss_row = row0, iss_l = 0;
    auto issue = [&](int slot) {
        const int col = iss_l * 512 + lane * 8;
        uint4 v = make_uint4(0, 0, 0, 0);
        if (col < p.k) v = zl_load_nt(reinterpret_cast<const uint4*>(p.w + (size_t)iss_row * p.k + col));
        wq[slot] = v;
        if (++iss_l == L) {
            iss_l = 0;
            ++iss_row;
        }
    };
#pragma unroll
    for (int s = 0; s < kRing; ++s)
        if (s < total) issue(s);

    zl_stage_rows<DT, MT, 256>(p.x, p.ldx, m0, p.m, p.k, p.kp, p.norm_w, p.norm_eps, xs, red);
    __syncthreads();

    float acc[MT];
    float best_v[MT];
    int best_i[MT];
#pragma unroll
    for (int m = 0; m < MT; ++m) {
        acc[m] = 0.f;
        best_v[m] = -INFINITY;
        best_i[m] = 0x7fffffff;
    }
    int cl = 0, crow = row0;
    auto consume = [&](int slot) {
#pragma unroll
        for (int m = 0; m < MT; ++m) {
            uint4 xa = *reinterpret_cast<const uint4*>(xs + (size_t)m * p.kp + cl * 512 + lane * 8);
            acc[m] = dot8<DT>(wq[slot], xa, acc[m]);
        }
        if (++cl == L) {
            cl = 0;
#pragma unroll
            for (int m = 0; m < MT; ++m) {
                float v = zl_wave_sum(acc[m]);
                acc[m] = 0.f;
                if (lane == 0 && (m0 + m) < p.m) {
                    float b = p.bias ? ZT<DT>::to_f32(p.bias[crow]) : 0.f;
                    const uint16_t y16 = ZT<DT>::from_f32(p.alpha * v + b);
                    p.y[(size_t)(m0 + m) * p.n + crow] = y16;
                    const float yv = ZT<DT>::to_f32(y16);
                    if (yv > best_v[m] || best_i[m] == 0x7fffffff || (yv != yv && best_v[m] == best_v[m])) {
                        best_v[m] = yv;
                        best_i[m] = crow;
                    }
                }
            }
            ++crow;
        }
    };
#pragma unroll 1
    for (int it = 0; it < total; it += kRing) {
#pragma unroll
        for (int s = 0; s < kRing; ++s) {
            if (it + s < total) {
                consume(s);
                if (it + s + kRing < total) issue(s);
            }
        }
    }
    if (p.argmax_ws && lane == 0) {
#pragma unroll
        for (int m = 0; m < MT; ++m)
            if ((m0 + m) < p.m)
                p.argmax_ws[(size_t)(m0 + m) * p.total_waves + gw] = make_float2(best_v[m], __int_as_float(best_i[m]));
    }
}

__device__ __forceinline__ bool greedy_beats(float v, int i, float bv, int bi) {
    if (i == 0x7fffffff) return false;
    if (bi == 0x7fffffff) return true;
    if (v != v) return bv == bv || i < bi;
    return v > bv || (v == bv && i < bi);
}

__global__ __launch_bounds__(256) void k_greedy_advance(const float2* ws, int total_waves, int32_t* tokens,
                                                        int32_t* positions, int32_t* placement, int32_t* valid_lens,
                                                        int64_t* next_out) {
    __shared__ float sv[256];
    __shared__ int si[256];
    const int b = blockIdx.x;
    float bv = -INFINITY;
    int bi = 0x7fffffff;
    for (int w0 = threadIdx.x; w0 < total_waves; w0 += 4 * 256) {
        float2 c[4];
#pragma unroll
        for (int u = 0; u < 4; ++u) {
            const int w = w0 + u * 256;
            c[u] = w < total_waves ? ws[(size_t)b * total_waves + w] : make_float2(0.f, __int_as_float(0x7fffffff));
        }
#pragma unroll
        for (int u = 0; u < 4; ++u) {
            const int ci = __float_as_int(c[u].y);
            if (greedy_beats(c[u].x, ci, bv, bi)) {
                bv = c[u].x;
                bi = ci;
            }
        }
    }
    sv[threadIdx.x] = bv;
    si[threadIdx.x] = bi;
    __syncthreads();
    for (int off = 128; off > 0; off >>= 1) {
        if ((int)threadIdx.x < off) {
            const float ov = sv[threadIdx.x + off];
            const int oi = si[threadIdx.x + off];
            if (greedy_beats(ov, oi, sv[threadIdx.x], si[threadIdx.x])) {
                sv[threadIdx.x] = ov;
                si[threadIdx.x] = oi;
            }
        }
        __syncthreads();
    }
    if (threadIdx.x == 0) {
        const int tok = si[0] == 0x7fffffff ? 0 : si[0];
        if (tokens) tokens[b] = tok;
        if (next_out) next_out[b] = tok;
        if (positions) positions[b] += 1;
        if (placement) placement[b] += 1;
        if (valid_lens) valid_lens[b] += 1;
    }
}

template <int DT, int MT>
int launch(const DenseParams& p, int gx, int gy, hipStream_t st) {
    size_t lds = (size_t)MT * p.kp * 2 + 64;
    if (lds > 160 * 1024) return ZL_ELIMIT;
    if (lds > 64 * 1024) {
        hipError_t e = hipFuncSetAttribute(reinterpret_cast<const void*>(&k_dense_gemv<DT, MT>),
                                           hipFuncAttributeMaxDynamicSharedMemorySize, (int)lds);
        if (e != hipSuccess) return (int)e;
    }
    hipLaunchKernelGGL((k_dense_gemv<DT, MT>), dim3(gx, gy), dim3(256), lds, st, p);
    return zl_launch_status();
}

template <int DT>
__global__ __launch_bounds__(64) void k_gemm_nt_f32(const uint16_t* __restrict__ x, int64_t ldx, const uint16_t* __restrict__ w, float* __restrict__ y,
                                                    int n, int k, float alpha) {
    const int col = blockIdx.x, row = blockIdx.y, lane = threadIdx.x;
    const uint16_t* xr = x + (int64_t)row * ldx;
    const uint16_t* wr = w + (int64_t)col * k;
    float acc = 0.f;
    for (int i = lane * 8; i + 8 <= k; i += 64 * 8) {
        const uint4 a = *reinterpret_cast<const uint4*>(xr + i), b = *reinterpret_cast<const uint4*>(wr + i);
        const uint32_t au[4] = {a.x, a.y, a.z, a.w}, bu[4] = {b.x, b.y, b.z, b.w};
#pragma unroll
        for (int e = 0; e < 4; ++e) {
            acc = __builtin_fmaf(ZT<DT>::to_f32((uint16_t)(au[e] & 0xffffu)), ZT<DT>::to_f32((uint16_t)(bu[e] & 0xffffu)), acc);
            acc = __builtin_fmaf(ZT<DT>::to_f32((uint16_t)(au[e] >> 16)), ZT<DT>::to_f32((uint16_t)(bu[e] >> 16)), acc);
        }
    }
    acc = zl_wave_sum(acc);
    if (lane == 0) y[(int64_t)row * n + col] = alpha * acc;
}

}

static int dense_waves(int64_t n, int* rows_per_wave, int* gx) {
    int cus = zl_device_cu_count();
    if (cus <= 0) cus = 256;
    const int waves = cus * 8;
    *rows_per_wave = (int)((n + waves - 1) / waves);
    *gx = (int)(((n + *rows_per_wave - 1) / *rows_per_wave + 3) / 4);
    return *gx * 4;
}

extern "C" int64_t zl_argmax_workspace_bytes(int64_t m, int64_t n) {
    if (m <= 0 || n <= 0) return ZL_EINVAL;
    int rpw, gx;
    return m * (int64_t)dense_waves(n, &rpw, &gx) * 8;
}

static int gemm_nt_small_m_impl(const uint16_t* x, int64_t ldx, const uint16_t* w, const uint16_t* bias, uint16_t* y,
                                int64_t m, int64_t n, int64_t k, float alpha, int dtype, const uint16_t* norm_weight,
                                float norm_eps, void* argmax_ws, zl_stream_t s) {
    ZL_CHECK_ARG(x && w && y && m > 0 && n > 0 && k > 0, ZL_EINVAL);
    ZL_CHECK_ARG(k % 8 == 0 && ldx % 8 == 0 && ldx >= k, ZL_ESHAPE);
    ZL_CHECK_ARG(dtype == ZL_F16 || dtype == ZL_BF16, ZL_EDTYPE);
    DenseParams p;
    p.x = x; p.ldx = ldx; p.w = w; p.bias = bias; p.y = y;
    p.norm_w = norm_weight; p.norm_eps = norm_eps; p.alpha = alpha;
    p.m = (int)m; p.n = (int)n; p.k = (int)k;
    p.kp = (int)((k + 511) / 512 * 512);
    p.loads_per_row = p.kp / 512;
    int mt = m >= 4 ? 4 : (int)m;
    while (mt > 1 && (size_t)mt * p.kp * 2 + 64 > 64 * 1024) --mt;
    if (mt == 3) mt = 2;
    const int gy = (int)((m + mt - 1) / mt);
    int gx;
    p.total_waves = dense_waves(n, &p.rows_per_wave, &gx);
    p.argmax_ws = reinterpret_cast<float2*>(argmax_ws);
    hipStream_t hs = (hipStream_t)s;
#define ZL_DISPATCH(DT)                                      \
    switch (mt) {                                            \
        case 1: return launch<DT, 1>(p, gx, gy, hs);         \
        case 2: return launch<DT, 2>(p, gx, gy, hs);         \
        default: return launch<DT, 4>(p, gx, gy, hs);        \
    }
    if (dtype == ZL_F16) { ZL_DISPATCH(ZL_F16) }
    ZL_DISPATCH(ZL_BF16)
#undef ZL_DISPATCH
}

extern "C" int zl_gemm_nt_small_m(const uint16_t* x, int64_t ldx, const uint16_t* w, const uint16_t* bias, uint16_t* y,
                                  int64_t m, int64_t n, int64_t k, float alpha, int dtype,
                                  const uint16_t* norm_weight, float norm_eps, zl_stream_t s) {
    return gemm_nt_small_m_impl(x, ldx, w, bias, y, m, n, k, alpha, dtype, norm_weight, norm_eps, nullptr, s);
}

extern "C" int zl_gemm_nt_small_m_argmax(const uint16_t* x, int64_t ldx, const uint16_t* w, const uint16_t* bias,
                                         uint16_t* y, int64_t m, int64_t n, int64_t k, float alpha, int dtype,
                                         const uint16_t* norm_weight, float norm_eps, void* argmax_ws, zl_stream_t s) {
    ZL_CHECK_ARG(argmax_ws, ZL_EINVAL);
    return gemm_nt_small_m_impl(x, ldx, w, bias, y, m, n, k, alpha, dtype, norm_weight, norm_eps, argmax_ws, s);
}

extern "C" int zl_gemm_nt_f32(const uint16_t* x, int64_t ldx, const uint16_t* w, float* y, int64_t m, int64_t n, int64_t k, float alpha, int dtype,
                              zl_stream_t s) {
    ZL_CHECK_ARG(x && w && y && m > 0 && n > 0 && k > 0, ZL_EINVAL);
    ZL_CHECK_ARG(k % 8 == 0 && ldx >= k && ldx % 8 == 0 && ((uintptr_t)x & 15) == 0 && ((uintptr_t)w & 15) == 0 && m <= 65535 && n < ((int64_t)1 << 31), ZL_ESHAPE);
    ZL_CHECK_ARG(dtype == ZL_F16 || dtype == ZL_BF16, ZL_EDTYPE);
    const dim3 grid((unsigned)n, (unsigned)m);
    if (dtype == ZL_F16) hipLaunchKernelGGL(k_gemm_nt_f32<ZL_F16>, grid, dim3(64), 0, (hipStream_t)s, x, ldx, w, y, (int)n, (int)k, alpha);
    else hipLaunchKernelGGL(k_gemm_nt_f32<ZL_BF16>, grid, dim3(64), 0, (hipStream_t)s, x, ldx, w, y, (int)n, (int)k, alpha);
    return zl_launch_status();
}

extern "C" int zl_greedy_advance(const void* argmax_ws, int64_t m, int64_t n, int32_t* tokens, int32_t* positions,
                                 int32_t* placement, int32_t* valid_lens, int64_t* next_tokens, zl_stream_t s) {
    ZL_CHECK_ARG(argmax_ws && m > 0 && n > 0, ZL_EINVAL);
    int rpw, gx;
    const int tw = dense_waves(n, &rpw, &gx);
    hipLaunchKernelGGL(k_greedy_advance, dim3((unsigned)m), dim3(256), 0, (hipStream_t)s,
                       reinterpret_cast<const float2*>(argmax_ws), tw, tokens, positions, placement, valid_lens, next_tokens);
    return zl_launch_status();
}
```

### zhilight_amd/csrc/w4_i8p.hip

```cpp
#include "zl_common.h"
#include "w4_i8p_common.h"

namespace {

constexpr int kT = 512, kW = 8;
#ifndef ZL_I8P_RING
#define ZL_I8P_RING 8
#endif
#ifndef ZL_I8P_EARLY
#define ZL_I8P_EARLY 0
#endif

#ifdef ZL_I8P_PROBE
__device__ unsigned long long* zl_probe_i8 = nullptr;
#define ZL_IPROBE_INIT()                                                                               \
    unsigned long long* pp_ = nullptr;                                                                 \
    if (zl_probe_i8 && (threadIdx.x & 63) == 0 && blockIdx.x < 2048)                                   \
        pp_ = zl_probe_i8 + ((size_t)blockIdx.x * kW + (threadIdx.x >> 6)) * 8;
#define ZL_IPROBE(slot)                                                                                \
    do {                                                                                               \
        if (pp_) pp_[slot] = wall_clock64();                                                           \
    } while (0)
#else
#define ZL_IPROBE_INIT() do {} while (0)
#define ZL_IPROBE(slot) do {} while (0)
#endif

template <int R, bool LONGK, bool ROPE, bool NORM, bool MERGE = false>
__global__ __launch_bounds__(kT, 2) void k_w4a16_i8p(const I8Params p) {
    static_assert(!ROPE || R == 2, "fused rotary: a tile and its partner tile");
    static_assert(!MERGE || (!LONGK && !ROPE && !NORM), "split merge: one column block, plain prologue");
    constexpr int XD = R >= ZL_I8P_RING ? 1 : (ZL_I8P_RING / R > 0 ? ZL_I8P_RING / R : 1);
    constexpr int D = R * XD;
    constexpr int NS = LONGK ? 8 : 4;
    constexpr int NR = LONGK ? 2 : 4;
    extern __shared__ __attribute__((aligned(16))) unsigned char smem[];
    ZL_IPROBE_INIT();
    ZL_IPROBE(0);
    const int lane = threadIdx.x & 63;
    const int wave = __builtin_amdgcn_readfirstlane(threadIdx.x >> 6);
    const int M = p.m, K = p.k, groups = p.groups;
    const int rec = 64 * M;
    const int Gw = (groups + kW - 1) / kW;
    unsigned char* planes = smem + (size_t)wave * Gw * 8 * rec;
    float* consts = reinterpret_cast<float*>(smem + (size_t)kW * Gw * 8 * rec) + (size_t)wave * Gw * 16;
    float* red = reinterpret_cast<float*>(smem + (size_t)kW * Gw * 8 * rec) + (size_t)kW * Gw * 16;
    float* scratch = red + R * kW * 64;

    const int tile0 = ROPE ? (blockIdx.x / p.pair_stride) * 2 * p.pair_stride + blockIdx.x % p.pair_stride : blockIdx.x * R;
    const int tile_stride = ROPE ? p.pair_stride : 1;
    const int my_groups = wave < groups ? (groups - wave + kW - 1) / kW : 0;

    constexpr int E = ZL_I8P_EARLY < D ? ZL_I8P_EARLY : D;
    uint4 wq[D];
    uint32_t mt[D];
    const __amdgpu_buffer_rsrc_t rq = __builtin_amdgcn_make_buffer_rsrc(const_cast<uint4*>(p.qw), 0, p.qw_bytes, 0x00020000);
    const __amdgpu_buffer_rsrc_t rm = __builtin_amdgcn_make_buffer_rsrc(const_cast<uint32_t*>(p.meta), 0, p.meta_bytes, 0x00020000);
    const __amdgpu_buffer_rsrc_t rnull = __builtin_amdgcn_make_buffer_rsrc(const_cast<uint4*>(p.qw), 0, 0, 0x00020000);
    const uint32_t q_off = (uint32_t)lane * 16u, m_off = (uint32_t)(lane & 15) * 4u;
    auto issue = [&](int slot, int gi, int r) {
        const int g = wave + kW * gi;
        const bool ok = g < groups;
        const uint32_t it = (uint32_t)(tile0 + r * tile_stride) * (uint32_t)groups + (uint32_t)g;
        wq[slot] = __builtin_bit_cast(uint4, __builtin_amdgcn_raw_buffer_load_b128(ok ? rq : rnull, q_off, it * 1024u, 2 ));
        mt[slot] = __builtin_amdgcn_raw_buffer_load_b32(ok ? rm : rnull, m_off, it * 64u, 2);
    };
    auto issue_early = [&]() {
        if constexpr (E > 0) {
            __builtin_amdgcn_sched_barrier(0);
#pragma unroll
            for (int q = 0; q < E; ++q) issue(q, q / R, q % R);
            __builtin_amdgcn_sched_barrier(0);
        }
    };

    uint4 xr[NS], nw[LONGK ? 4 : 1];
    const int lgi = lane >> 4, uo = lane & 15;
#pragma unroll
    for (int c = 0; c < (LONGK ? 4 : 1); ++c) {
        nw[c] = make_uint4(0, 0, 0, 0);
        const int g = wave + kW * (4 * c + lgi);
        if (NORM && 4 * c < Gw) nw[c] = *reinterpret_cast<const uint4*>(p.norm_w + (g < groups ? g * 128 + uo * 8 : 0));
    }
#pragma unroll
    for (int s = 0; s < NS; ++s) {
        const int row = LONGK ? (s & 1) : s, c = LONGK ? (s >> 1) : 0;
        const int g = wave + kW * (4 * c + lgi);
        xr[s] = make_uint4(0, 0, 0, 0);
        if constexpr (MERGE) {
            if (row < M) {
                constexpr int kS = 16;
                const int head = g < groups ? g : 0;
                const uint32_t n_rec = (uint32_t)M * (uint32_t)groups * (uint32_t)p.mg_max_splits;
                const __amdgpu_buffer_rsrc_t rpart = __builtin_amdgcn_make_buffer_rsrc(const_cast<uint16_t*>(p.mg_part), 0, n_rec * 256u, 0x00020000);
                const __amdgpu_buffer_rsrc_t rstat = __builtin_amdgcn_make_buffer_rsrc(const_cast<float*>(p.mg_stat), 0, n_rec * 8u, 0x00020000);
                const uint32_t rec0 = ((uint32_t)row * (uint32_t)groups + (uint32_t)head) * (uint32_t)p.mg_max_splits;
                const uint32_t po = rec0 * 256u + (uint32_t)uo * 16u, so = rec0 * 8u;
                uint4 pv[kS];
                float2 st[kS];
#pragma unroll
                for (int u = 0; u < kS; ++u) {
                    const uint32_t uc = u < p.mg_max_splits ? (uint32_t)u : 0u;
                    pv[u] = __builtin_bit_cast(uint4, __builtin_amdgcn_raw_buffer_load_b128(rpart, po, uc * 256u, 0));
                    st[u] = __builtin_bit_cast(float2, __builtin_amdgcn_raw_buffer_load_b64(rstat, so, uc * 8u, 0));
                }
                if (s == 0) issue_early();
                const int elen = min(p.buf_lens[row], p.mg_valid_lens[row]);
                const int ns = min((elen + p.mg_split_len - 1) / p.mg_split_len, kS);
                float mn = -1e20f;
#pragma unroll
                for (int u = 0; u < kS; ++u) mn = fmaxf(mn, u < ns ? st[u].x : -1e20f);
                float a[8] = {0.f, 0.f, 0.f, 0.f, 0.f, 0.f, 0.f, 0.f}, z = 0.f;
#pragma unroll
                for (int u = 0; u < kS; ++u) {
                    if (u < ns) {
                        const float f = st[u].y * __expf(st[u].x - mn);
                        const uint32_t w4[4] = {pv[u].x, pv[u].y, pv[u].z, pv[u].w};
#pragma unroll
                        for (int e = 0; e < 4; ++e) {
                            const h16x2 hh = __builtin_bit_cast(h16x2, w4[e]);
                            a[2 * e] = __builtin_fmaf((float)hh.x, f, a[2 * e]);
                            a[2 * e + 1] = __builtin_fmaf((float)hh.y, f, a[2 * e + 1]);
                        }
                        z += f;
                    }
                }
                const float zi = 1.0f / (z + 1e-20f);
                uint32_t o[4];
#pragma unroll
                for (int e = 0; e < 4; ++e) {
                    h16x2 hh;
                    hh.x = zl_f32_to_f16(a[2 * e] * zi);
                    hh.y = zl_f32_to_f16(a[2 * e + 1] * zi);
                    o[e] = __builtin_bit_cast(uint32_t, hh);
                }
                if (g < groups) xr[s] = make_uint4(o[0], o[1], o[2], o[3]);
            }
        } else
        if (row < M && 4 * c < Gw) {
            xr[s] = *reinterpret_cast<const uint4*>(p.x + (g < groups ? (size_t)row * p.ldx + g * 128 + uo * 8 : 0));
            if (g >= groups) xr[s] = make_uint4(0, 0, 0, 0);
        }
    }
    ZlRopeOperands rp;
    if constexpr (ROPE) {
        if ((int)threadIdx.x < 16 * M) rp = zl_rope_prefetch(p, threadIdx.x >> 4, tile0 * 16 + (threadIdx.x & 15));
    }
    const bool silu = (p.epi & (ZL_EPI_SILU_MUL | ZL_EPI_SILU_MUL_F32)) != 0;
    float ep_b0 = 0.f, ep_b1 = 0.f, ep_res = 0.f, ep_prev = 0.f;
    int ep_r = 0, ep_m = 0, ep_nl = 0, ep_col = -1;
    if constexpr (!ROPE) {
        const int per_tile = (silu ? 8 : 16) * M;
        if ((int)threadIdx.x < R * per_tile) {
            ep_r = threadIdx.x / per_tile;
            const int rem = threadIdx.x % per_tile, tile = tile0 + ep_r;
            if (!silu) {
                ep_m = rem >> 4; ep_nl = rem & 15;
                const int row = tile * 16 + ep_nl;
                if (tile < p.tiles && row < p.n) {
                    ep_col = row;
                    if ((p.epi & ZL_EPI_BIAS) && p.bias) ep_b0 = (float)__builtin_bit_cast(_Float16, p.bias[row]);
                    if (p.epi & ZL_EPI_ADD_C) ep_prev = (float)__builtin_bit_cast(_Float16, p.y[(size_t)ep_m * p.ld_out + row]);
                    if (p.epi & ZL_EPI_RESIDUAL) ep_res = (float)__builtin_bit_cast(_Float16, p.residual[(size_t)ep_m * p.ld_out + row]);
                }
            } else {
                ep_m = rem >> 3; ep_nl = rem & 7;
                const int pr = tile * 8 + ep_nl;
                if (tile < p.tiles && 2 * pr + 1 < p.n) {
                    ep_col = pr;
                    if ((p.epi & ZL_EPI_BIAS) && p.bias) {
                        ep_b0 = (float)__builtin_bit_cast(_Float16, p.bias[2 * pr]);
                        ep_b1 = (float)__builtin_bit_cast(_Float16, p.bias[2 * pr + 1]);
                    }
                }
            }
        }
    }
    if constexpr (!MERGE) issue_early();
    __builtin_amdgcn_sched_barrier(0);
    static_assert(2 * E < 16, "vmcnt immediate");
    __builtin_amdgcn_s_waitcnt(0x0F70 | (2 * E));
    __builtin_amdgcn_sched_barrier(0);
    ZL_IPROBE(1);

#define ZL_ISSUE_RANGE(LO, HI)                                     \
    {                                                              \
        __builtin_amdgcn_sched_barrier(0);                         \
        _Pragma("unroll") for (int q = ((LO) > E ? (LO) : E); q < (HI); ++q) issue(q, q / R, q % R); \
        __builtin_amdgcn_sched_barrier(0);                         \
    }
    constexpr int Q0 = NORM ? D / 2 : 0, NP = LONGK ? 8 : 4;
#define ZL_QLO(pos) (Q0 + ((D - Q0) * (pos) + NP - 1) / NP)

    float rs[NR];
#pragma unroll
    for (int r = 0; r < NR; ++r) rs[r] = 1.f;
    if constexpr (NORM) {
        float part[NR];
#pragma unroll
        for (int r = 0; r < NR; ++r) part[r] = 0.f;
#pragma unroll
        for (int s = 0; s < NS; ++s) {
            const int row = LONGK ? (s & 1) : s;
            const uint32_t u[4] = {xr[s].x, xr[s].y, xr[s].z, xr[s].w};
#pragma unroll
            for (int e = 0; e < 4; ++e) {
                const h16x2 hh = __builtin_bit_cast(h16x2, u[e]);
                part[row] = __builtin_fmaf((float)hh.x, (float)hh.x, part[row]);
                part[row] = __builtin_fmaf((float)hh.y, (float)hh.y, part[row]);
            }
        }
#pragma unroll
        for (int r = 0; r < NR; ++r) {
            if (r < M) {
                const float t = wave_sum_hi(part[r]);
                if (lane == 63) scratch[r * kW + wave] = t;
            }
        }
        ZL_ISSUE_RANGE(0, Q0)
        __syncthreads();
        const bool pow2 = (K & (K - 1)) == 0;
        const float inv_k = 1.0f / (float)K;
#pragma unroll
        for (int r = 0; r < NR; ++r) {
            if (r < M) {
                float tot = 0.f;
#pragma unroll
                for (int w = 0; w < kW; ++w) tot += scratch[r * kW + w];
                rs[r] = zl_rsqrt_rn((pow2 ? tot * inv_k : tot / (float)K) + p.norm_eps);
            }
        }
    }
    ZL_IPROBE(2);

#pragma unroll
    for (int s = 0; s < NS; ++s) {
        const int row = LONGK ? (s & 1) : s, c = LONGK ? (s >> 1) : 0;
        if (row < M && 4 * c < Gw) {
            const int gi = 4 * c + lgi;
            const bool live = wave + kW * gi < groups;
            uint32_t u[4] = {xr[s].x, xr[s].y, xr[s].z, xr[s].w};
            if constexpr (NORM) {
                const uint32_t wu[4] = {nw[c].x, nw[c].y, nw[c].z, nw[c].w};
#pragma unroll
                for (int e = 0; e < 4; ++e) {
                    const h16x2 hh = __builtin_bit_cast(h16x2, u[e]), ww = __builtin_bit_cast(h16x2, wu[e]);
                    h16x2 o;
                    o.x = zl_f32_to_f16((float)hh.x * rs[row] * (float)ww.x);
                    o.y = zl_f32_to_f16((float)hh.y * rs[row] * (float)ww.y);
                    u[e] = __builtin_bit_cast(uint32_t, o);
                }
            }
            typedef unsigned short us2 __attribute__((ext_vector_type(2)));
            const us2 m01 = __builtin_elementwise_max(__builtin_bit_cast(us2, u[0] & 0x7fff7fffu), __builtin_bit_cast(us2, u[1] & 0x7fff7fffu));
            const us2 m23 = __builtin_elementwise_max(__builtin_bit_cast(us2, u[2] & 0x7fff7fffu), __builtin_bit_cast(us2, u[3] & 0x7fff7fffu));
            const us2 mm = __builtin_elementwise_max(m01, m23);
            int am = max((int)mm.x, (int)mm.y);
            am = row16_max(am);
            if (row == 0 && c < NP / 4) ZL_ISSUE_RANGE(ZL_QLO(4 * c + 0), ZL_QLO(4 * c + 1))
            const int ef = min(am >> 10, 30);
            const float up = __builtin_bit_cast(float, (uint32_t)(163 - ef) << 23);
            const float xscale = am >= 0x7c00 ? __builtin_bit_cast(float, 0x7fc00000u) : __builtin_bit_cast(float, (uint32_t)(91 + ef) << 23);
            uint32_t Y[8];
#pragma unroll
            for (int e = 0; e < 4; ++e) {
                const h16x2 hh = __builtin_bit_cast(h16x2, u[e]);
                Y[2 * e] = (uint32_t)__builtin_fmaf((float)hh.x, up, 8421504.f);
                Y[2 * e + 1] = (uint32_t)__builtin_fmaf((float)hh.y, up, 8421504.f);
            }
            int sx = (int)(((Y[0] + Y[1]) + (Y[2] + Y[3])) + ((Y[4] + Y[5]) + (Y[6] + Y[7]))) - 8 * 0x808080;
            sx = row16_sum(sx);
            if (row == 0 && c < NP / 4) ZL_ISSUE_RANGE(ZL_QLO(4 * c + 1), ZL_QLO(4 * c + 2))
            auto planes_of = [&](int i0, int i1, int i2, int i3, uint32_t& d2, uint32_t& d1, uint32_t& d0) {
                const uint32_t P = __builtin_amdgcn_perm(Y[i1], Y[i0], 0x05010400u);
                const uint32_t Q = __builtin_amdgcn_perm(Y[i3], Y[i2], 0x05010400u);
                const uint32_t P2 = __builtin_amdgcn_perm(Y[i1], Y[i0], 0x0c0c0602u);
                const uint32_t Q2 = __builtin_amdgcn_perm(Y[i3], Y[i2], 0x0c0c0602u);
                d0 = __builtin_amdgcn_perm(Q, P, 0x05040100u) ^ 0x80808080u;
                d1 = __builtin_amdgcn_perm(Q, P, 0x07060302u) ^ 0x80808080u;
                d2 = __builtin_amdgcn_perm(Q2, P2, 0x05040100u) ^ 0x80808080u;
            };
            uint32_t a2, a1, a0, b2, b1, b0;
            planes_of(0, 4, 1, 5, a2, a1, a0);
            planes_of(2, 6, 3, 7, b2, b1, b0);
            if (row == 0 && c < NP / 4) ZL_ISSUE_RANGE(ZL_QLO(4 * c + 2), ZL_QLO(4 * c + 3))
            unsigned char* dst = planes + (size_t)((gi * 2 + (uo >> 3)) * 4 + (uo & 3)) * rec + (size_t)(4 * row) * 16 + ((uo >> 2) & 1) * 8;
            if (live) {
                *reinterpret_cast<uint2*>(dst) = make_uint2(a2, b2);
                *reinterpret_cast<uint2*>(dst + 16) = make_uint2(a1, b1);
                *reinterpret_cast<uint2*>(dst + 32) = make_uint2(a0, b0);
                if (row == 0) *reinterpret_cast<uint2*>(dst + 48) = make_uint2(0, 0);
                if (uo == 0) {
                    const float bx = xscale * (float)sx;
                    *reinterpret_cast<float4*>(consts + ((size_t)gi * 4 + row) * 4) = make_float4(xscale, 65536.f * xscale, bx, 1024.f * bx);
                }
            }
            if (row == 0 && c < NP / 4) ZL_ISSUE_RANGE(ZL_QLO(4 * c + 3), ZL_QLO(4 * c + 4))
        }
    }
#undef ZL_ISSUE_RANGE
#undef ZL_QLO
    asm volatile("s_waitcnt lgkmcnt(0)" ::: "memory");
    __builtin_amdgcn_wave_barrier();
    ZL_IPROBE(3);

    const int kq = lane >> 4, row16 = lane & 15;
    const int aslot = (row16 < 4 * M && (row16 & 3) != 3) ? row16 : 3;
    const unsigned char* a_base = planes + (size_t)kq * rec + aslot * 16;
    const int crow = min(kq, M - 1);
    float acc[R];
#pragma unroll
    for (int r = 0; r < R; ++r) acc[r] = 0.f;
    const uint32_t m4 = __builtin_amdgcn_readfirstlane(0x0f0f0f0fu);
    const v4i zero4 = (v4i){0, 0, 0, 0};

    for (int gi0 = 0; gi0 < my_groups; gi0 += XD) {
#pragma unroll
        for (int j = 0; j < XD; ++j) {
            const int gi = gi0 + j;
            if (j > 0 && gi >= my_groups) break;
            const v4i a0 = *reinterpret_cast<const v4i*>(a_base + (size_t)(gi * 2 + 0) * 4 * rec);
            const v4i a1 = *reinterpret_cast<const v4i*>(a_base + (size_t)(gi * 2 + 1) * 4 * rec);
            const float4 cst = *reinterpret_cast<const float4*>(consts + ((size_t)gi * 4 + crow) * 4);
#pragma unroll
            for (int r = 0; r < R; ++r) {
                const int slot = j * R + r;
                const uint4 w = wq[slot];
                const uint32_t mw = mt[slot];
                v4i b0, b1;
                b0[0] = (int)(w.x & m4); b0[1] = (int)((w.x >> 4) & m4); b0[2] = (int)(w.y & m4); b0[3] = (int)((w.y >> 4) & m4);
                b1[0] = (int)(w.z & m4); b1[1] = (int)((w.z >> 4) & m4); b1[2] = (int)(w.w & m4); b1[3] = (int)((w.w >> 4) & m4);
                v4i d = __builtin_amdgcn_mfma_i32_16x16x64_i8(a0, b0, zero4, 0, 0, 0);
                d = __builtin_amdgcn_mfma_i32_16x16x64_i8(a1, b1, d, 0, 0, 0);
                issue(slot, gi + XD, r);
                const h16x2 sm = __builtin_bit_cast(h16x2, mw);
                const float f12 = (float)((d[1] << 8) + d[2]), f0 = (float)d[0];
                float t = __builtin_fmaf((float)sm.y, cst.z, cst.w);
                t = __builtin_fmaf(f12, cst.x, t);
                t = __builtin_fmaf(f0, cst.y, t);
                asm volatile("" : "+v"(t) : "v"(b0), "v"(b1), "v"(a0), "v"(a1));
                acc[r] = __builtin_fmaf((float)sm.x, t, acc[r]);
#ifdef ZL_I8P_PROBE
                if (gi == 0 && r == 0) ZL_IPROBE(4);
#endif
            }
        }
    }

    ZL_IPROBE(5);
#pragma unroll
    for (int r = 0; r < R; ++r) red[(r * kW + wave) * 64 + lane] = acc[r];
    __syncthreads();
    ZL_IPROBE(6);
    auto total_of = [&](int r, int n_local, int m) {
        float v = 0.f;
#pragma unroll
        for (int w = 0; w < kW; ++w) v += red[(r * kW + w) * 64 + m * 16 + n_local];
        return v;
    };
    if constexpr (ROPE) {
        if ((int)threadIdx.x < 16 * M) {
            const int m = threadIdx.x >> 4, n_local = threadIdx.x & 15;
            zl_rope_store_f16(p, rp, m, tile0 * 16 + n_local, total_of(0, n_local, m), total_of(1, n_local, m));
        }
        ZL_IPROBE(7);
        return;
    }
    if (ep_col >= 0) {
        if (!silu) {
            const _Float16 y16 = zl_w4m_finish(total_of(ep_r, ep_nl, ep_m), ep_b0, ep_prev, ep_res, p.epi);
            p.y[(size_t)ep_m * p.ld_out + ep_col] = __builtin_bit_cast(uint16_t, y16);
        } else {
            const float g = total_of(ep_r, 2 * ep_nl, ep_m) + ep_b0, u = total_of(ep_r, 2 * ep_nl + 1, ep_m) + ep_b1;
            p.y[(size_t)ep_m * p.ld_out + ep_col] = __builtin_bit_cast(uint16_t, zl_f32_to_f16(zl_w4m_finish_gated(g, u, p.epi)));
        }
    }
    ZL_IPROBE(7);
}

static size_t i8p_lds_bytes(int groups, int m, int r) {
    const size_t gw = (groups + kW - 1) / kW;
    return kW * gw * 8 * 64 * (size_t)m + kW * gw * 64 + (size_t)r * kW * 64 * 4 + 4 * kW * 4;
}

template <int R, bool LONGK, bool ROPE, bool NORM, bool MERGE = false>
int launch_i8p_n(const I8Params& p, int grid, hipStream_t hs) {
    const size_t lds = i8p_lds_bytes(p.groups, p.m, R);
    if (lds > 160 * 1024) return ZL_ELIMIT;
    if (lds > 64 * 1024) {
        hipError_t e = hipFuncSetAttribute(reinterpret_cast<const void*>(&k_w4a16_i8p<R, LONGK, ROPE, NORM, MERGE>),
                                           hipFuncAttributeMaxDynamicSharedMemorySize, (int)lds);
        if (e != hipSuccess) return ZL_ELIMIT;
    }
    hipLaunchKernelGGL((k_w4a16_i8p<R, LONGK, ROPE, NORM, MERGE>), dim3(grid), dim3(kT), lds, hs, p);
    return zl_launch_status();
}
template <int R, bool ROPE>
int launch_i8p(const I8Params& p, int grid, hipStream_t hs) {
    const bool lk = p.groups > 4 * kW;
    if (p.norm_w) return lk ? launch_i8p_n<R, true, ROPE, true>(p, grid, hs) : launch_i8p_n<R, false, ROPE, true>(p, grid, hs);
    return lk ? launch_i8p_n<R, true, ROPE, false>(p, grid, hs) : launch_i8p_n<R, false, ROPE, false>(p, grid, hs);
}

}

#ifdef ZL_I8P_PROBE
extern "C" int zl_debug_set_probe_i8p(void* p) { return (int)hipMemcpyToSymbol(HIP_SYMBOL(zl_probe_i8), &p, sizeof(p)); }
#endif

bool zl_w4a16_i8p_covers(int64_t m, int64_t k) {
    if (m < 1 || m > 4 || k < 128 || k % 128 != 0 || k > 16384 || (k > 4096 && m > 2)) return false;
    return i8p_lds_bytes((int)(k / 128), (int)m, 8) <= 160 * 1024;
}

int zl_w4a16_gemm_i8p(const W4Problem& pb, int rounds_override, hipStream_t hs) {
    if (!zl_w4a16_i8p_covers(pb.m, pb.k)) return ZL_ESHAPE;
    const I8Params p = i8_params(pb);
    const int cus = zl_cu_count();
    int r = (pb.tiles + cus - 1) / cus;
    if (r > 8) r = 8;
    if (rounds_override > 0 && rounds_override <= 8) r = rounds_override;
    const int grid = (pb.tiles + r - 1) / r;
#define ZL_I8(RR) case RR: return launch_i8p<RR, false>(p, grid, hs);
    switch (r) { ZL_I8(1) ZL_I8(2) ZL_I8(3) ZL_I8(4) ZL_I8(5) ZL_I8(6) ZL_I8(7) ZL_I8(8) }
#undef ZL_I8
    return ZL_EINVAL;
}

int zl_w4a16_gemm_i8p_rope(const W4Problem& pb, const W4Rope& rp, hipStream_t hs) {
    if (!zl_w4a16_i8p_covers(pb.m, pb.k) || !zl_w4m_rope_shape_ok(pb, rp)) return ZL_ESHAPE;
    I8Params p = i8_params(pb);
    i8_fill_rope(p, rp);
    return launch_i8p<2, true>(p, pb.tiles / 2, hs);
}

int zl_w4a16_gemm_i8p_merge(const W4Problem& pb, const W4Merge& mg, hipStream_t hs) {
    if (pb.m < 1 || pb.m > 4 || pb.k > 4096 || pb.k % 128 != 0 || mg.max_splits < 1 || mg.max_splits > 16 || mg.split_len < 1) return ZL_ESHAPE;
    if (pb.epilogue & (ZL_EPI_SILU_MUL | ZL_EPI_SILU_MUL_F32)) return ZL_ESHAPE;
    I8Params p = i8_params(pb);
    i8_fill_merge(p, mg);
    const int cus = zl_cu_count();
    int r = (pb.tiles + cus - 1) / cus;
    if (r > 8) r = 8;
    const int grid = (pb.tiles + r - 1) / r;
#define ZL_I8M(RR) case RR: return launch_i8p_n<RR, false, false, false, true>(p, grid, hs);
    switch (r) { ZL_I8M(1) ZL_I8M(2) ZL_I8M(3) ZL_I8M(4) ZL_I8M(5) ZL_I8M(6) ZL_I8M(7) ZL_I8M(8) }
#undef ZL_I8M
    return ZL_EINVAL;
}
```

Before: 649.8 tokens/s.

## Preload hot kernel arguments into SGPRs and add a single-chunk decode attention path

Enables the AMDGPU kernarg preload flag for the i8p GEMV, attention and dense GEMV sources. It also moves the fields each kernel reads first out of the params struct into leading scalar arguments, so they can be preloaded into SGPRs instead of loaded from kernarg memory at kernel start. Attention gains a single-chunk specialization for when split_len equals one chunk: it drops the prefetch loop, uses global address-space pointers and issues the Q load early with schedule barriers. The i8p kernel moves its vmcnt wait ahead of the epilogue operand loads and keeps those operands as raw bits to shorten prologue latency. The changes add extra kernel arguments and a getenv call on every attention launch.

```diff
diff --git a/zhilight_amd/build.py b/zhilight_amd/build.py
--- a/zhilight_amd/build.py
+++ b/zhilight_amd/build.py
@@ -10,6 +10,13 @@
 FLAGS = ["--offload-arch=gfx950", "-O3", "-std=c++17", "-fPIC", "-Wall", "-Wno-unused-function",
          "-fno-fast-math", "-ffp-contract=off"]
 EXTRA_FLAGS = {"w4_slab.hip": ["-mllvm", "-pragma-unroll-threshold=200000"]}
+KERNARG_PRELOAD = os.environ.get("ZL_KERNARG_PRELOAD", "1") != "0"
+PRELOAD_FLAGS = ["-mllvm", "-amdgpu-kernarg-preload-count=16"]
+PRELOAD_SOURCES = ("w4_i8p.hip", "attention.hip", "dense_gemv.hip")
+
+
+def extra_flags(name):
+    return EXTRA_FLAGS.get(name, []) + (PRELOAD_FLAGS if KERNARG_PRELOAD and name in PRELOAD_SOURCES else [])
 
 
 EXPERIMENTAL = os.environ.get("ZL_BUILD_EXPERIMENTAL", "0") == "1"
@@ -38,7 +45,8 @@
     os.makedirs(objdir, exist_ok=True)
     flags = FLAGS + (["-DZL_EXPERIMENTAL", "-I" + CSRC] if EXPERIMENTAL else [])
     stamp = os.path.join(objdir, ".flags")
-    if not os.path.exists(stamp) or open(stamp).read() != " ".join(flags):
+    stamp_text = " ".join(flags + ["preload" if KERNARG_PRELOAD else "no-preload"])
+    if not os.path.exists(stamp) or open(stamp).read() != stamp_text:
         force = True
     objs = []
     jobs = []
@@ -46,7 +54,7 @@
         o = os.path.join(objdir, os.path.basename(s)[:-4] + ".o")
         objs.append(o)
         if force or _stale(o, [s] + hdrs):
-            jobs.append([HIPCC] + flags + EXTRA_FLAGS.get(os.path.basename(s), []) + ["-c", s, "-o", o])
+            jobs.append([HIPCC] + flags + extra_flags(os.path.basename(s)) + ["-c", s, "-o", o])
 
     def run(cmd):
         if verbose:
@@ -58,7 +66,7 @@
     if jobs or force or _stale(OUT, objs):
         run([HIPCC, "--offload-arch=gfx950", "-shared", "-fPIC", "-o", OUT] + objs)
     with open(stamp, "w") as fh:
-        fh.write(" ".join(flags))
+        fh.write(stamp_text)
     build_hostcpp(force, verbose)
     build_comm(force, verbose)
     _ref().build(force, verbose)
diff --git a/zhilight_amd/csrc/attention.hip b/zhilight_amd/csrc/attention.hip
--- a/zhilight_amd/csrc/attention.hip
+++ b/zhilight_amd/csrc/attention.hip
@@ -1,4 +1,5 @@
 #include <algorithm>
+#include <cstdlib>
 #include <type_traits>
 #include "zl_common.h"
 
@@ -732,46 +733,55 @@
 #define ZL_ATTN8_WAVES_PER_SIMD 2
 #endif
 #define ZL_ATTN8_OCC(NW_) ((NW_) == 4 ? 4 : ZL_ATTN8_WAVES_PER_SIMD)
-template <int DT, int NW = 4, bool LA = false, int PF = 1, bool MASKED = false, bool CAUSAL = false>
-__global__ __launch_bounds__(64 * NW, PF >= 3 ? 1 : (PF == 2 || MASKED) ? 2 : ZL_ATTN8_OCC(NW)) void k_decode_attn_mfma(const AttnParams p) {
+template <int DT, int NW = 4, bool LA = false, int PF = 1, bool MASKED = false, bool CAUSAL = false, bool ONE = false>
+__global__ __launch_bounds__(64 * NW, PF >= 3 ? 1 : (PF == 2 || MASKED) ? 2 : ZL_ATTN8_OCC(NW)) void k_decode_attn_mfma(
+    const uint16_t* hq, const int32_t* hbuf_lens, const uint16_t* const* hk_bufs, const uint16_t* const* hv_bufs, const void* hvis,
+    const unsigned hsplit_bshd, const int hhkv, const unsigned hlenq_nrep, const AttnParams p) {
+    static_assert(!ONE || (!LA && PF == 1 && !CAUSAL), "the single-chunk form exists for the two-launch route only");
+    const int split_len = (int)(hsplit_bshd >> 1), bshd = (int)(hsplit_bshd & 1u), hkv = hhkv;
+    const int n_rep = (int)(hlenq_nrep & 0xffffu), len_q = (int)(hlenq_nrep >> 16), rows = len_q * n_rep, nh = hkv * n_rep;
+    const int32_t* valid_lens = reinterpret_cast<const int32_t*>(hvis);
     static_assert(!MASKED || (!LA && PF == 1), "the mask form exists for the two-launch route only");
     static_assert(!CAUSAL || (!LA && PF == 1 && !MASKED && NW == 4), "the causal form exists for the two-launch route only");
     __shared__ __attribute__((aligned(16))) uint16_t vs[NW][32 * kMVS];
-    const int b = blockIdx.z, hk = CAUSAL ? (int)(blockIdx.y % (unsigned)p.hkv) : (int)blockIdx.y, split = blockIdx.x;
-    const int row0 = CAUSAL ? 16 * (int)(blockIdx.y / (unsigned)p.hkv) : 0;
-    const int nrows = CAUSAL ? min(16, p.rows - row0) : p.rows;
-    const int len = p.buf_lens[b];
-    const int vlen_in = MASKED ? 0x7fffffff : CAUSAL ? p.valid_lens[b] + (row0 + nrows - 1) / p.n_rep : p.valid_lens[b];
+    const int b = blockIdx.z, hk = CAUSAL ? (int)(blockIdx.y % (unsigned)hkv) : (int)blockIdx.y, split = blockIdx.x;
+    const int row0 = CAUSAL ? 16 * (int)(blockIdx.y / (unsigned)hkv) : 0;
+    const int nrows = CAUSAL ? min(16, rows - row0) : rows;
+    const int len = hbuf_lens[b];
+    const int vlen_in = MASKED ? 0x7fffffff : CAUSAL ? valid_lens[b] + (row0 + nrows - 1) / n_rep : valid_lens[b];
     const int8_t* mrow = nullptr;
     if constexpr (MASKED) {
         size_t mask_off = 0;
-        for (int i = 0; i < b; ++i) mask_off += (size_t)p.buf_lens[i];
-        mrow = p.mask + mask_off;
-    }
-    const uint16_t* kbase = p.k_bufs[b];
-    const uint16_t* vbase = p.v_bufs[b];
+        for (int i = 0; i < b; ++i) mask_off += (size_t)hbuf_lens[i];
+        mrow = reinterpret_cast<const int8_t*>(hvis) + mask_off;
+    }
+    typedef std::conditional_t<ONE, const __attribute__((address_space(1))) uint16_t*, const uint16_t*> kv_ptr;
+    typedef uint32_t kv_u4 __attribute__((ext_vector_type(4)));
+    typedef std::conditional_t<ONE, const __attribute__((address_space(1))) kv_u4*, const kv_u4*> kv_ptr4;
+    const kv_ptr kbase = (kv_ptr)hk_bufs[b];
+    const kv_ptr vbase = (kv_ptr)hv_bufs[b];
     const int elen = min(len, vlen_in);
-    const int t0 = split * p.split_len;
+    const int t0 = split * split_len;
     const int nw = LA ? __builtin_amdgcn_readfirstlane((int)(blockDim.x >> 6)) : NW;
     ZL_APROBE_INIT();
     ZL_APROBE(0);
     if (t0 >= elen || len <= 0) {
         if constexpr (LA) {
             if (split == 0)
-                for (int idx = threadIdx.x; idx < p.rows * kMD; idx += nw * 64) {
-                    const int i = idx / kMD, qi = i / p.n_rep, head = hk * p.n_rep + i % p.n_rep;
-                    p.out[(((size_t)b * p.len_q + qi) * p.h + head) * kMD + idx % kMD] = 0;
+                for (int idx = threadIdx.x; idx < rows * kMD; idx += nw * 64) {
+                    const int i = idx / kMD, qi = i / n_rep, head = hk * n_rep + i % n_rep;
+                    p.out[(((size_t)b * len_q + qi) * nh + head) * kMD + idx % kMD] = 0;
                 }
         }
         return;
     }
-    const int t1 = min(elen, t0 + p.split_len);
+    const int t1 = min(elen, t0 + split_len);
     const int last_key = t1 - 1;
 
     const int lane = threadIdx.x & 63, wave = threadIdx.x >> 6;
     const int r = lane & 15, kq = lane >> 4;
-    const size_t kv_stride = p.bshd ? (size_t)p.hkv * kMD : (size_t)kMD;
-    const size_t kv_off = p.bshd ? (size_t)hk * kMD : (size_t)hk * len * kMD;
+    const size_t kv_stride = bshd ? (size_t)hkv * kMD : (size_t)kMD;
+    const size_t kv_off = bshd ? (size_t)hk * kMD : (size_t)hk * len * kMD;
 
     uint4 kkA[2][4], kkB[PF >= 2 ? 2 : 1][4], kkC[PF >= 3 ? 2 : 1][4];
     uint4 vA0, vA1, vA2, vA3, vA4, vA5, vA6, vA7, vB0, vB1, vB2, vB3, vB4, vB5, vB6, vB7, vC0, vC1, vC2, vC3, vC4, vC5, vC6, vC7;
@@ -780,13 +790,13 @@
 #define ZL_MFMA_LOAD_K(KK, base)                                                                                  \
     _Pragma("unroll") for (int blk_ = 0; blk_ < 2; ++blk_) {                                                   \
         const int key_ = (base) + 16 * blk_ + r;                                                               \
-        const uint16_t* src_ = kbase + kv_off + (size_t)(key_ < last_key ? key_ : last_key) * kv_stride + 8 * kq; \
-        _Pragma("unroll") for (int t_ = 0; t_ < 4; ++t_) KK[blk_][t_] = *reinterpret_cast<const uint4*>(src_ + 32 * t_); \
+        const kv_ptr src_ = kbase + kv_off + (size_t)(key_ < last_key ? key_ : last_key) * kv_stride + 8 * kq; \
+        _Pragma("unroll") for (int t_ = 0; t_ < 4; ++t_) KK[blk_][t_] = __builtin_bit_cast(uint4, *(kv_ptr4)(src_ + 32 * t_)); \
     }
 #define ZL_MFMA_V1(VS, j_, base)                                                                                 \
     {                                                                                                          \
         const int key_ = (base) + 4 * j_ + (lane >> 4);                                                        \
-        VS##j_ = *reinterpret_cast<const uint4*>(vbase + kv_off + (size_t)(key_ < last_key ? key_ : last_key) * kv_stride + (lane & 15) * 8); \
+        VS##j_ = __builtin_bit_cast(uint4, *(kv_ptr4)(vbase + kv_off + (size_t)(key_ < last_key ? key_ : last_key) * kv_stride + (lane & 15) * 8)); \
     }
 #define ZL_MFMA_LOAD_V(VS, base)                                                                               \
     ZL_MFMA_V1(VS, 0, base) ZL_MFMA_V1(VS, 1, base) ZL_MFMA_V1(VS, 2, base) ZL_MFMA_V1(VS, 3, base) ZL_MFMA_V1(VS, 4, base) \
@@ -797,9 +807,30 @@
         const int key_ = (base) + (lane & 31);                                                                 \
         MB = mrow[key_ < last_key ? key_ : last_key];                                                          \
     }
+    uint4 qf[4];
+    int rlim = t1;
+    auto load_q = [&]() __attribute__((always_inline)) {
+        uint4 z = make_uint4(0, 0, 0, 0);
+        const bool live = r < nrows;
+        const int rr = row0 + (live ? r : 0);
+        const int qi = rr / n_rep, head = hk * n_rep + rr % n_rep;
+        if constexpr (CAUSAL) rlim = min(t1, valid_lens[b] + qi);
+        const uint16_t* qp = hq + (((size_t)b * len_q + qi) * nh + head) * kMD + 8 * kq;
+#pragma unroll
+        for (int t = 0; t < 4; ++t) {
+            uint4 v = *reinterpret_cast<const uint4*>(qp + 32 * t);
+            qf[t] = live ? v : z;
+        }
+    };
     ZL_MFMA_LOAD_M(mbA, c0)
+    if constexpr (ONE) {
+        load_q();
+        __builtin_amdgcn_sched_barrier(0);
+    }
     ZL_MFMA_LOAD_K(kkA, c0)
+    if constexpr (ONE) __builtin_amdgcn_sched_barrier(0);
     ZL_MFMA_LOAD_V(vA, c0)
+    if constexpr (ONE) __builtin_amdgcn_sched_barrier(0);
     if constexpr (PF >= 2) {
         ZL_MFMA_LOAD_K(kkB, c0 + cstep)
         ZL_MFMA_LOAD_V(vB, c0 + cstep)
@@ -810,21 +841,7 @@
     }
     ZL_APROBE(1);
 
-    uint4 qf[4];
-    int rlim = t1;
-    {
-        uint4 z = make_uint4(0, 0, 0, 0);
-        const bool live = r < nrows;
-        const int rr = row0 + (live ? r : 0);
-        const int qi = rr / p.n_rep, head = hk * p.n_rep + rr % p.n_rep;
-        if constexpr (CAUSAL) rlim = min(t1, p.valid_lens[b] + qi);
-        const uint16_t* qp = p.q + (((size_t)b * p.len_q + qi) * p.h + head) * kMD + 8 * kq;
-#pragma unroll
-        for (int t = 0; t < 4; ++t) {
-            uint4 v = *reinterpret_cast<const uint4*>(qp + 32 * t);
-            qf[t] = live ? v : z;
-        }
-    }
+    if constexpr (!ONE) load_q();
 
     f4v o[8];
 #pragma unroll
@@ -839,11 +856,14 @@
         uint32_t vbits = 0xffffffffu;
         if constexpr (MASKED) {
             vbits = (uint32_t)__ballot(lane < 32 && MB != 0 && cur + lane < t1);
+        }
+        auto zero_invisible_v = [&]() __attribute__((always_inline)) {
             const int vsh = lane >> 4;
 #define ZL_MFMA_VZ(j_) if (!((vbits >> (4 * j_ + vsh)) & 1u)) v##j_ = make_uint4(0, 0, 0, 0);
             ZL_MFMA_VZ(0) ZL_MFMA_VZ(1) ZL_MFMA_VZ(2) ZL_MFMA_VZ(3) ZL_MFMA_VZ(4) ZL_MFMA_VZ(5) ZL_MFMA_VZ(6) ZL_MFMA_VZ(7)
 #undef ZL_MFMA_VZ
-        }
+        };
+        if constexpr (MASKED && !ONE) zero_invisible_v();
         f4v st[2];
 #pragma unroll
         for (int blk = 0; blk < 2; ++blk) {
@@ -851,6 +871,10 @@
 #pragma unroll
             for (int t = 0; t < 4; ++t)
                 st[blk] = mfma_t<DT>(KK[blk][t], qf[t], st[blk]);
+        }
+        if constexpr (ONE) {
+            __builtin_amdgcn_sched_barrier(0);
+            if constexpr (MASKED) zero_invisible_v();
         }
         {
             uint16_t* vdst = vsw + (lane >> 4) * kMVS + (lane & 15) * 8;
@@ -858,9 +882,11 @@
             ZL_MFMA_VST(0) ZL_MFMA_VST(1) ZL_MFMA_VST(2) ZL_MFMA_VST(3) ZL_MFMA_VST(4) ZL_MFMA_VST(5) ZL_MFMA_VST(6) ZL_MFMA_VST(7)
 #undef ZL_MFMA_VST
         }
-        ZL_MFMA_LOAD_M(MB, cur + PF * cstep)
-        ZL_MFMA_LOAD_K(KK, cur + PF * cstep)
-        ZL_MFMA_LOAD_V(v, cur + PF * cstep)
+        if constexpr (!ONE) {
+            ZL_MFMA_LOAD_M(MB, cur + PF * cstep)
+            ZL_MFMA_LOAD_K(KK, cur + PF * cstep)
+            ZL_MFMA_LOAD_V(v, cur + PF * cstep)
+        }
         float sv[2][4];
         float mloc = -INFINITY;
 #pragma unroll
@@ -924,6 +950,9 @@
             o[db] = mfma_t<DT>(__builtin_bit_cast(uint4, a), pl, o[db]);
         }
     };
+    if constexpr (ONE) {
+        if (c0 >= 0) chunk(kkA, vA0, vA1, vA2, vA3, vA4, vA5, vA6, vA7, mbA, c0);
+    } else
     while (c0 >= 0) {
         chunk(kkA, vA0, vA1, vA2, vA3, vA4, vA5, vA6, vA7, mbA, c0);
         c0 += cstep;
@@ -962,9 +991,9 @@
     if constexpr (LA) {
         ZL_APROBE(4);
 #ifdef ZL_ATTN_PROBE
-        attn_tail_la<DT>(p, xw, b, hk, split, nw, (elen + p.split_len - 1) / p.split_len, ap_);
+        attn_tail_la<DT>(p, xw, b, hk, split, nw, (elen + split_len - 1) / split_len, ap_);
 #else
-        attn_tail_la<DT>(p, xw, b, hk, split, nw, (elen + p.split_len - 1) / p.split_len, nullptr);
+        attn_tail_la<DT>(p, xw, b, hk, split, nw, (elen + split_len - 1) / split_len, nullptr);
 #endif
         return;
     }
@@ -982,13 +1011,13 @@
             a = __builtin_fmaf(src[w * WS + d], f, a);
             lt = __builtin_fmaf(src[w * WS + kMD + 1], f, lt);
         }
-        const int qi = (row0 + i) / p.n_rep, head = hk * p.n_rep + (row0 + i) % p.n_rep;
-        const size_t rec = (((size_t)b * p.len_q + qi) * p.h + head) * p.max_splits + split;
+        const int qi = (row0 + i) / n_rep, head = hk * n_rep + (row0 + i) % n_rep;
+        const size_t rec = (((size_t)b * len_q + qi) * nh + head) * p.max_splits + split;
         if (p.half_partials) {
             uint16_t* hp = reinterpret_cast<uint16_t*>(p.ws);
             hp[rec * kMD + d] = __builtin_bit_cast(uint16_t, (_Float16)((MASKED && lt == 0.f) ? 0.f : a / lt));
             if (d == 0) {
-                float* st = p.ws + (size_t)p.b * p.len_q * p.h * p.max_splits * (kMD / 2) + rec * 2;
+                float* st = p.ws + (size_t)p.b * len_q * nh * p.max_splits * (kMD / 2) + rec * 2;
                 st[0] = mn;
                 st[1] = lt;
             }
@@ -1326,8 +1355,24 @@
 int launch_mfma(const AttnParams& p, int dtype, hipStream_t st, int waves = NW) {
     const int tiles = CAUSAL ? (p.rows + 15) / 16 : 1;
     const dim3 grid((unsigned)p.max_splits, (unsigned)(p.hkv * tiles), (unsigned)p.b);
+    bool one = false;
+    if constexpr (!LA && PF == 1 && !CAUSAL) {
+        const char* sw = getenv("ZL_ATTN_ONE_CHUNK");
+        one = p.split_len == 32 * NW && waves == NW && !(sw && sw[0] == '0');
+    }
+    if (p.len_q > 0xffff || p.n_rep > 0xffff) return ZL_ELIMIT;
+    const unsigned split_bshd = ((unsigned)p.split_len << 1) | (p.bshd ? 1u : 0u), lenq_nrep = ((unsigned)p.len_q << 16) | (unsigned)p.n_rep;
+    const void* vis = MASKED ? (const void*)p.mask : (const void*)p.valid_lens;
     return by_dtype(dtype, [&](auto dt) {
-        hipLaunchKernelGGL((k_decode_attn_mfma<decltype(dt)::value, NW, LA, PF, MASKED, CAUSAL>), grid, dim3(64 * waves), 0, st, p);
+        if constexpr (!LA && PF == 1 && !CAUSAL) {
+            if (one) {
+                hipLaunchKernelGGL((k_decode_attn_mfma<decltype(dt)::value, NW, LA, PF, MASKED, CAUSAL, true>), grid, dim3(64 * waves), 0, st, p.q,
+                                   p.buf_lens, p.k_bufs, p.v_bufs, vis, split_bshd, p.hkv, lenq_nrep, p);
+                return zl_launch_status();
+            }
+        }
+        hipLaunchKernelGGL((k_decode_attn_mfma<decltype(dt)::value, NW, LA, PF, MASKED, CAUSAL>), grid, dim3(64 * waves), 0, st, p.q, p.buf_lens,
+                           p.k_bufs, p.v_bufs, vis, split_bshd, p.hkv, lenq_nrep, p);
         return zl_launch_status();
     });
 }
diff --git a/zhilight_amd/csrc/dense_gemv.hip b/zhilight_amd/csrc/dense_gemv.hip
--- a/zhilight_amd/csrc/dense_gemv.hip
+++ b/zhilight_amd/csrc/dense_gemv.hip
@@ -39,19 +39,21 @@
 }
 
 template <int DT, int MT>
-__global__ __launch_bounds__(256) void k_dense_gemv(const DenseParams p) {
+__global__ __launch_bounds__(256) void k_dense_gemv(const uint16_t* hw, const uint16_t* hx, const uint16_t* hnorm_w, const int64_t hldx, const int hk,
+                                                    const int hn, const int hrows_per_wave, const int hloads_per_row, const int hm, const int hkp,
+                                                    const DenseParams p) {
     extern __shared__ __attribute__((aligned(16))) unsigned char smem[];
     uint16_t* xs = reinterpret_cast<uint16_t*>(smem);
-    float* red = reinterpret_cast<float*>(smem + (size_t)MT * p.kp * 2);
+    float* red = reinterpret_cast<float*>(smem + (size_t)MT * hkp * 2);
 
     const int lane = threadIdx.x & 63;
     const int wave = __builtin_amdgcn_readfirstlane(threadIdx.x >> 6);
     const int m0 = blockIdx.y * MT;
-    const int L = p.loads_per_row;
+    const int L = hloads_per_row;
     const int gw = blockIdx.x * 4 + wave;
-    const int row0 = gw * p.rows_per_wave;
-    int nrows = p.n - row0;
-    nrows = nrows < 0 ? 0 : (nrows > p.rows_per_wave ? p.rows_per_wave : nrows);
+    const int row0 = gw * hrows_per_wave;
+    int nrows = hn - row0;
+    nrows = nrows < 0 ? 0 : (nrows > hrows_per_wave ? hrows_per_wave : nrows);
     const int total = nrows * L;
 
     uint4 wq[kRing];
@@ -59,7 +61,7 @@
     auto issue = [&](int slot) {
         const int col = iss_l * 512 + lane * 8;
         uint4 v = make_uint4(0, 0, 0, 0);
-        if (col < p.k) v = zl_load_nt(reinterpret_cast<const uint4*>(p.w + (size_t)iss_row * p.k + col));
+        if (col < hk) v = zl_load_nt(reinterpret_cast<const uint4*>(hw + (size_t)iss_row * hk + col));
         wq[slot] = v;
         if (++iss_l == L) {
             iss_l = 0;
@@ -70,7 +72,7 @@
     for (int s = 0; s < kRing; ++s)
         if (s < total) issue(s);
 
-    zl_stage_rows<DT, MT, 256>(p.x, p.ldx, m0, p.m, p.k, p.kp, p.norm_w, p.norm_eps, xs, red);
+    zl_stage_rows<DT, MT, 256>(hx, hldx, m0, hm, hk, hkp, hnorm_w, p.norm_eps, xs, red);
     __syncthreads();
 
     float acc[MT];
@@ -86,7 +88,7 @@
     auto consume = [&](int slot) {
 #pragma unroll
         for (int m = 0; m < MT; ++m) {
-            uint4 xa = *reinterpret_cast<const uint4*>(xs + (size_t)m * p.kp + cl * 512 + lane * 8);
+            uint4 xa = *reinterpret_cast<const uint4*>(xs + (size_t)m * hkp + cl * 512 + lane * 8);
             acc[m] = dot8<DT>(wq[slot], xa, acc[m]);
         }
         if (++cl == L) {
@@ -95,10 +97,10 @@
             for (int m = 0; m < MT; ++m) {
                 float v = zl_wave_sum(acc[m]);
                 acc[m] = 0.f;
-                if (lane == 0 && (m0 + m) < p.m) {
+                if (lane == 0 && (m0 + m) < hm) {
                     float b = p.bias ? ZT<DT>::to_f32(p.bias[crow]) : 0.f;
                     const uint16_t y16 = ZT<DT>::from_f32(p.alpha * v + b);
-                    p.y[(size_t)(m0 + m) * p.n + crow] = y16;
+                    p.y[(size_t)(m0 + m) * hn + crow] = y16;
                     const float yv = ZT<DT>::to_f32(y16);
                     if (yv > best_v[m] || best_i[m] == 0x7fffffff || (yv != yv && best_v[m] == best_v[m])) {
                         best_v[m] = yv;
@@ -122,7 +124,7 @@
     if (p.argmax_ws && lane == 0) {
 #pragma unroll
         for (int m = 0; m < MT; ++m)
-            if ((m0 + m) < p.m)
+            if ((m0 + m) < hm)
                 p.argmax_ws[(size_t)(m0 + m) * p.total_waves + gw] = make_float2(best_v[m], __int_as_float(best_i[m]));
     }
 }
@@ -191,7 +193,8 @@
                                            hipFuncAttributeMaxDynamicSharedMemorySize, (int)lds);
         if (e != hipSuccess) return (int)e;
     }
-    hipLaunchKernelGGL((k_dense_gemv<DT, MT>), dim3(gx, gy), dim3(256), lds, st, p);
+    hipLaunchKernelGGL((k_dense_gemv<DT, MT>), dim3(gx, gy), dim3(256), lds, st, p.w, p.x, p.norm_w, p.ldx, p.k, p.n, p.rows_per_wave,
+                       p.loads_per_row, p.m, p.kp, p);
     return zl_launch_status();
 }
 
diff --git a/zhilight_amd/csrc/w4_i8p.hip b/zhilight_amd/csrc/w4_i8p.hip
--- a/zhilight_amd/csrc/w4_i8p.hip
+++ b/zhilight_amd/csrc/w4_i8p.hip
@@ -27,7 +27,9 @@
 #endif
 
 template <int R, bool LONGK, bool ROPE, bool NORM, bool MERGE = false>
-__global__ __launch_bounds__(kT, 2) void k_w4a16_i8p(const I8Params p) {
+__global__ __launch_bounds__(kT, 2) void k_w4a16_i8p(const uint16_t* hx, const void* haux, const int32_t* hlen0, const int32_t* hlen1,
+                                                     const int64_t hldx, const int hm, const int hgroups, const int hsplits, const int hsplit_len,
+                                                     const I8Params p) {
     static_assert(!ROPE || R == 2, "fused rotary: a tile and its partner tile");
     static_assert(!MERGE || (!LONGK && !ROPE && !NORM), "split merge: one column block, plain prologue");
     constexpr int XD = R >= ZL_I8P_RING ? 1 : (ZL_I8P_RING / R > 0 ? ZL_I8P_RING / R : 1);
@@ -39,7 +41,7 @@
     ZL_IPROBE(0);
     const int lane = threadIdx.x & 63;
     const int wave = __builtin_amdgcn_readfirstlane(threadIdx.x >> 6);
-    const int M = p.m, K = p.k, groups = p.groups;
+    const int M = hm, groups = hgroups;
     const int rec = 64 * M;
     const int Gw = (groups + kW - 1) / kW;
     unsigned char* planes = smem + (size_t)wave * Gw * 8 * rec;
@@ -80,7 +82,7 @@
     for (int c = 0; c < (LONGK ? 4 : 1); ++c) {
         nw[c] = make_uint4(0, 0, 0, 0);
         const int g = wave + kW * (4 * c + lgi);
-        if (NORM && 4 * c < Gw) nw[c] = *reinterpret_cast<const uint4*>(p.norm_w + (g < groups ? g * 128 + uo * 8 : 0));
+        if (NORM && 4 * c < Gw) nw[c] = *reinterpret_cast<const uint4*>(reinterpret_cast<const uint16_t*>(haux) + (g < groups ? g * 128 + uo * 8 : 0));
     }
 #pragma unroll
     for (int s = 0; s < NS; ++s) {
@@ -91,22 +93,22 @@
             if (row < M) {
                 constexpr int kS = 16;
                 const int head = g < groups ? g : 0;
-                const uint32_t n_rec = (uint32_t)M * (uint32_t)groups * (uint32_t)p.mg_max_splits;
-                const __amdgpu_buffer_rsrc_t rpart = __builtin_amdgcn_make_buffer_rsrc(const_cast<uint16_t*>(p.mg_part), 0, n_rec * 256u, 0x00020000);
-                const __amdgpu_buffer_rsrc_t rstat = __builtin_amdgcn_make_buffer_rsrc(const_cast<float*>(p.mg_stat), 0, n_rec * 8u, 0x00020000);
-                const uint32_t rec0 = ((uint32_t)row * (uint32_t)groups + (uint32_t)head) * (uint32_t)p.mg_max_splits;
+                const uint32_t n_rec = (uint32_t)M * (uint32_t)groups * (uint32_t)hsplits;
+                const __amdgpu_buffer_rsrc_t rpart = __builtin_amdgcn_make_buffer_rsrc(const_cast<uint16_t*>(hx), 0, n_rec * 256u, 0x00020000);
+                const __amdgpu_buffer_rsrc_t rstat = __builtin_amdgcn_make_buffer_rsrc(const_cast<void*>(haux), 0, n_rec * 8u, 0x00020000);
+                const uint32_t rec0 = ((uint32_t)row * (uint32_t)groups + (uint32_t)head) * (uint32_t)hsplits;
                 const uint32_t po = rec0 * 256u + (uint32_t)uo * 16u, so = rec0 * 8u;
                 uint4 pv[kS];
                 float2 st[kS];
 #pragma unroll
                 for (int u = 0; u < kS; ++u) {
-                    const uint32_t uc = u < p.mg_max_splits ? (uint32_t)u : 0u;
+                    const uint32_t uc = u < hsplits ? (uint32_t)u : 0u;
                     pv[u] = __builtin_bit_cast(uint4, __builtin_amdgcn_raw_buffer_load_b128(rpart, po, uc * 256u, 0));
                     st[u] = __builtin_bit_cast(float2, __builtin_amdgcn_raw_buffer_load_b64(rstat, so, uc * 8u, 0));
                 }
                 if (s == 0) issue_early();
-                const int elen = min(p.buf_lens[row], p.mg_valid_lens[row]);
-                const int ns = min((elen + p.mg_split_len - 1) / p.mg_split_len, kS);
+                const int elen = min(hlen0[row], hlen1[row]);
+                const int ns = min((elen + hsplit_len - 1) / hsplit_len, kS);
                 float mn = -1e20f;
 #pragma unroll
                 for (int u = 0; u < kS; ++u) mn = fmaxf(mn, u < ns ? st[u].x : -1e20f);
@@ -138,16 +140,23 @@
             }
         } else
         if (row < M && 4 * c < Gw) {
-            xr[s] = *reinterpret_cast<const uint4*>(p.x + (g < groups ? (size_t)row * p.ldx + g * 128 + uo * 8 : 0));
+            xr[s] = *reinterpret_cast<const uint4*>(hx + (g < groups ? (size_t)row * hldx + g * 128 + uo * 8 : 0));
             if (g >= groups) xr[s] = make_uint4(0, 0, 0, 0);
         }
     }
+    if constexpr (!MERGE) issue_early();
+    __builtin_amdgcn_sched_barrier(0);
+    static_assert(2 * E < 16, "vmcnt immediate");
+    __builtin_amdgcn_s_waitcnt(0x0F70 | (2 * E));
+    __builtin_amdgcn_sched_barrier(0);
+    ZL_IPROBE(1);
+    const int K = p.k;
     ZlRopeOperands rp;
     if constexpr (ROPE) {
         if ((int)threadIdx.x < 16 * M) rp = zl_rope_prefetch(p, threadIdx.x >> 4, tile0 * 16 + (threadIdx.x & 15));
     }
     const bool silu = (p.epi & (ZL_EPI_SILU_MUL | ZL_EPI_SILU_MUL_F32)) != 0;
-    float ep_b0 = 0.f, ep_b1 = 0.f, ep_res = 0.f, ep_prev = 0.f;
+    uint32_t ep_b0 = 0, ep_b1 = 0, ep_res = 0, ep_prev = 0;
     int ep_r = 0, ep_m = 0, ep_nl = 0, ep_col = -1;
     if constexpr (!ROPE) {
         const int per_tile = (silu ? 8 : 16) * M;
@@ -159,9 +168,9 @@
                 const int row = tile * 16 + ep_nl;
                 if (tile < p.tiles && row < p.n) {
                     ep_col = row;
-                    if ((p.epi & ZL_EPI_BIAS) && p.bias) ep_b0 = (float)__builtin_bit_cast(_Float16, p.bias[row]);
-                    if (p.epi & ZL_EPI_ADD_C) ep_prev = (float)__builtin_bit_cast(_Float16, p.y[(size_t)ep_m * p.ld_out + row]);
-                    if (p.epi & ZL_EPI_RESIDUAL) ep_res = (float)__builtin_bit_cast(_Float16, p.residual[(size_t)ep_m * p.ld_out + row]);
+                    if ((p.epi & ZL_EPI_BIAS) && p.bias) ep_b0 = p.bias[row];
+                    if (p.epi & ZL_EPI_ADD_C) ep_prev = p.y[(size_t)ep_m * p.ld_out + row];
+                    if (p.epi & ZL_EPI_RESIDUAL) ep_res = p.residual[(size_t)ep_m * p.ld_out + row];
                 }
             } else {
                 ep_m = rem >> 3; ep_nl = rem & 7;
@@ -169,19 +178,14 @@
                 if (tile < p.tiles && 2 * pr + 1 < p.n) {
                     ep_col = pr;
                     if ((p.epi & ZL_EPI_BIAS) && p.bias) {
-                        ep_b0 = (float)__builtin_bit_cast(_Float16, p.bias[2 * pr]);
-                        ep_b1 = (float)__builtin_bit_cast(_Float16, p.bias[2 * pr + 1]);
+                        ep_b0 = p.bias[2 * pr];
+                        ep_b1 = p.bias[2 * pr + 1];
                     }
                 }
             }
         }
     }
-    if constexpr (!MERGE) issue_early();
     __builtin_amdgcn_sched_barrier(0);
-    static_assert(2 * E < 16, "vmcnt immediate");
-    __builtin_amdgcn_s_waitcnt(0x0F70 | (2 * E));
-    __builtin_amdgcn_sched_barrier(0);
-    ZL_IPROBE(1);
 
 #define ZL_ISSUE_RANGE(LO, HI)                                     \
     {                                                              \
@@ -367,11 +371,15 @@
         return;
     }
     if (ep_col >= 0) {
+        auto f16 = [](uint32_t bits) {
+            asm volatile("" : "+v"(bits));
+            return (float)__builtin_bit_cast(_Float16, (uint16_t)bits);
+        };
         if (!silu) {
-            const _Float16 y16 = zl_w4m_finish(total_of(ep_r, ep_nl, ep_m), ep_b0, ep_prev, ep_res, p.epi);
+            const _Float16 y16 = zl_w4m_finish(total_of(ep_r, ep_nl, ep_m), f16(ep_b0), f16(ep_prev), f16(ep_res), p.epi);
             p.y[(size_t)ep_m * p.ld_out + ep_col] = __builtin_bit_cast(uint16_t, y16);
         } else {
-            const float g = total_of(ep_r, 2 * ep_nl, ep_m) + ep_b0, u = total_of(ep_r, 2 * ep_nl + 1, ep_m) + ep_b1;
+            const float g = total_of(ep_r, 2 * ep_nl, ep_m) + f16(ep_b0), u = total_of(ep_r, 2 * ep_nl + 1, ep_m) + f16(ep_b1);
             p.y[(size_t)ep_m * p.ld_out + ep_col] = __builtin_bit_cast(uint16_t, zl_f32_to_f16(zl_w4m_finish_gated(g, u, p.epi)));
         }
     }
@@ -392,7 +400,12 @@
                                            hipFuncAttributeMaxDynamicSharedMemorySize, (int)lds);
         if (e != hipSuccess) return ZL_ELIMIT;
     }
-    hipLaunchKernelGGL((k_w4a16_i8p<R, LONGK, ROPE, NORM, MERGE>), dim3(grid), dim3(kT), lds, hs, p);
+    if constexpr (MERGE)
+        hipLaunchKernelGGL((k_w4a16_i8p<R, LONGK, ROPE, NORM, MERGE>), dim3(grid), dim3(kT), lds, hs, p.mg_part, (const void*)p.mg_stat, p.buf_lens,
+                           p.mg_valid_lens, p.ldx, p.m, p.groups, p.mg_max_splits, p.mg_split_len, p);
+    else
+        hipLaunchKernelGGL((k_w4a16_i8p<R, LONGK, ROPE, NORM, MERGE>), dim3(grid), dim3(kT), lds, hs, p.x, (const void*)p.norm_w, (const int32_t*)nullptr,
+                           (const int32_t*)nullptr, p.ldx, p.m, p.groups, 0, 0, p);
     return zl_launch_status();
 }
 template <int R, bool ROPE>
```

Result: no change. 656.1 tokens/s, median of 6 (+1.0%).
